# totokunda/apex-studio

Measured on AMD Instinct MI355X. Metric: denoise_steps_per_sec, higher is better.
Workload: dtype bf16; 1 GPU; flux-dev-1024x1024 denoise step (19 double + 38 single MM-DiT blocks, S_img 4096 + S_txt 512, B=1, no CFG) + FlowMatch-Euler step; clips_in_flight=1, parallelism=clip-per-gpu x1

## Files before the change

### apex-studio_amd/build.py

```python
from __future__ import annotations

import hashlib
import os
import shutil
import subprocess
import sys

PKG_DIR = os.path.dirname(os.path.abspath(__file__))
CSRC = os.path.join(PKG_DIR, "csrc")
LIB_NAME = "libapex_mi355.so"
LIB_PATH = os.path.join(PKG_DIR, LIB_NAME)
SOURCES = ["runtime.hip", "gemm.hip", "attention.hip", "attention_masked.hip", "elementwise.hip", "conv.hip"]
ARCH = "gfx950"


def _hipcc() -> str:
    for cand in (os.environ.get("HIPCC"), shutil.which("hipcc"), "/opt/rocm/bin/hipcc"):
        if cand and os.path.exists(cand):
            return cand
    raise RuntimeError("hipcc not found (set HIPCC or install ROCm)")


FLAGS = ["-O3", "-std=c++17", "-fPIC", "-Wno-unused-result"]
if os.environ.get("APEXMI_GEMM_STREAMK", "0") not in ("", "0"):
    FLAGS.append("-DAPEXMI_GEMM_STREAMK=1")
if os.environ.get("APEXMI_DEBUG", "0") not in ("", "0"):
    FLAGS.append("-DAPEXMI_DEBUG")


NO_SPILL = {"attention.hip": ["attn_fwd_d128_w64_kernel", "attn_fwd_d128_w64r_kernel"],
            "attention_masked.hip": ["attn_masked_kernel"]}
REMARKS = "-Rpass-analysis=kernel-resource-usage"


def parse_resource_remarks(text: str) -> dict:
    import re
    out, cur = {}, None
    for line in text.splitlines():
        m = re.search(r"remark:\s+Function Name: (\S+)", line)
        if m:
            cur = out.setdefault(m.group(1), {})
            continue
        m = re.search(r"remark:\s+([A-Za-z ]+?)(?: \[[^\]]*\])?: (\d+)", line)
        if m and cur is not None:
            cur[m.group(1).strip()] = int(m.group(2))
    return out


def check_no_spill(src: str, remarks: str) -> None:
    res = parse_resource_remarks(remarks)
    for want in NO_SPILL.get(src, []):
        hits = {k: v for k, v in res.items() if want in k}
        if not hits:
            raise RuntimeError(f"build: no resource remark for kernel '{want}' of {src} — the spill check cannot run")
        for k, v in hits.items():
            bad = {f: v.get(f, -1) for f in ("ScratchSize", "SGPRs Spill", "VGPRs Spill") if v.get(f, -1) != 0}
            if bad:
                raise RuntimeError(f"build: {k} ({src}) has a hand-fixed register map and must not spill, but the compiler "
                                   f"reports {bad} (VGPRs {v.get('VGPRs')}, AGPRs {v.get('AGPRs')}, SGPRs {v.get('TotalSGPRs')}): "
                                   f"this hipcc allocates differently from the one the map was written against")


def _digest(paths: list[str], extra: str = "") -> str:
    h = hashlib.sha256(extra.encode())
    for p in paths:
        with open(p, "rb") as f:
            h.update(hashlib.sha256(f.read()).digest())
    return h.hexdigest()


def _stale(target: str, digest: str) -> bool:
    stamp = target + ".sha256"
    if not (os.path.exists(target) and os.path.exists(stamp)):
        return True
    with open(stamp) as f:
        return f.read().strip() != digest


def _stamp(target: str, digest: str) -> None:
    with open(target + ".sha256", "w") as f:
        f.write(digest + "\n")


def build(force: bool = False, verbose: bool = True) -> str:
    hipcc = _hipcc()
    headers = [os.path.join(CSRC, "common.h"),
               os.path.join(PKG_DIR, "..", "include", "apexmi.h")]
    headers += sorted(os.path.join(CSRC, f) for f in os.listdir(CSRC) if f.endswith((".inc", ".h")) and f != "common.h")
    objs = []
    jobs = []
    for src in SOURCES:
        sp = os.path.join(CSRC, src)
        op = os.path.join(CSRC, src.replace(".hip", ".o"))
        objs.append(op)
        dg = _digest([sp] + headers, " ".join(FLAGS + ([REMARKS + ":checked"] if src in NO_SPILL else []) + [ARCH]))
        if force or _stale(op, dg):
            cmd = [hipcc, f"--offload-arch={ARCH}", *FLAGS, *([REMARKS] if src in NO_SPILL else []), "-c", sp, "-o", op]
            if verbose:
                print("[build]", " ".join(cmd), flush=True)
            jobs.append((subprocess.Popen(cmd, stderr=subprocess.PIPE if src in NO_SPILL else None, text=True), cmd, op, dg, src))
    for proc, cmd, op, dg, src in jobs:
        err = proc.communicate()[1]
        if err:
            rest = [l for l in err.splitlines() if "kernel-resource-usage" not in l and not l.lstrip().startswith(("|", "^"))
                    and not l.strip()[:1].isdigit() and not l.startswith("In file included from")]
            if rest and verbose:
                print("\n".join(rest), file=sys.stderr, flush=True)
        if proc.returncode != 0:
            if err:
                print(err[-4000:], file=sys.stderr)
            raise subprocess.CalledProcessError(proc.returncode, cmd)
        if src in NO_SPILL:
            check_no_spill(src, err or "")
        _stamp(op, dg)
    dg = _digest(objs, ARCH)
    if force or _stale(LIB_PATH, dg):
        cmd = [hipcc, f"--offload-arch={ARCH}", "-shared", "-fPIC", "-o", LIB_PATH] + objs
        if verbose:
            print("[build]", " ".join(cmd), flush=True)
        subprocess.check_call(cmd)
        _stamp(LIB_PATH, dg)
    return LIB_PATH


if __name__ == "__main__":
    build(force="--force" in sys.argv)
    print(LIB_PATH)
```

### apex-studio_amd/csrc/gemm.hip

```cpp
#include "common.h"

#include <cstring>
#include <mutex>
#include <tuple>
#include <type_traits>
#include <vector>

namespace {

#ifndef APEXMI_GEMM_ABLATE
#define APEXMI_GEMM_ABLATE 0
#endif
#ifndef APEXMI_GEMM_PEEL
#define APEXMI_GEMM_PEEL 2
#endif
#ifndef APEXMI_GEMM_STREAMK
#define APEXMI_GEMM_STREAMK 0
#endif
#ifndef APEXMI_GEMM_TRACE
#define APEXMI_GEMM_TRACE 0
#endif
constexpr int BK = 64;
constexpr int GROUP_M = 6;
constexpr int EPI_GATE_RES_F32 = 7;
constexpr int MAX_GROUPS = 4;

struct GemmProblem {
    const bf16_t* A;
    const bf16_t* W;
    const bf16_t* bias;
    bf16_t* C;
    const float* gate;
    const bf16_t* R;
    int64_t lda, ldw, ldc, ldr;
    int M, N, nm, nn, tile0, gelu;
    int qkv, row0;
    const bf16_t* nq;
    const bf16_t* nk;
};
struct QkvShared {
    bf16_t* qo;
    bf16_t* ko;
    bf16_t* vt;
    const float* rope;
    int S_out, Skp, inner;
    float eps;
    const float* rope_pairs;
};
struct GemmGroup {
    GemmProblem p[MAX_GROUPS];
    int count, K, total, group_m;
    int batch;
    int64_t bsA, bsW, bsC_bytes;
    QkvShared qs;
    unsigned long long* clk;
#if APEXMI_GEMM_TRACE
    unsigned long long* trace;
#endif
    int wpacked;
    int sk_r, sk_tfull;
    float* sk_slab;
    unsigned* sk_flag;
};
enum { TILE_FULL = 0, TILE_WRITER = 1, TILE_OWNER = 2 };
struct SkCtx {
    int mode, kt0, kt1;
    int cu;
    int nparts;
};

template <int BM_, int BN_, int WM_, int WN_, int SCHED_>
struct Cfg {
    static constexpr int BM = BM_, BN = BN_, WM = WM_, WN = WN_;
    static constexpr int SCHED = SCHED_;
    static constexpr bool PP = SCHED_ == 1;
    static constexpr int NW = WM * WN, NT = NW * 64;
    static constexpr int TM = BM / WM / 32, TN = BN / WN / 32;
    static constexpr int A_BYTES = BM * BK * 2, W_BYTES = BN * BK * 2;
    static constexpr int STAGE = A_BYTES + W_BYTES;
    static constexpr int LDS = SCHED_ == 8 ? 5 * 32768 : 2 * STAGE;
    static constexpr int A_LD = BM * 8 / NT, W_LD = BN * 8 / NT;
    static constexpr int OCC = (LDS <= 80 * 1024 && NT == 256) ? 2 : (NT == 512 ? 2 : 1);
};
using CFG_128 = Cfg<128, 128, 2, 2, 0>;
using CFG_256 = Cfg<256, 256, 2, 4, 0>;
using CFG_128E = Cfg<128, 128, 2, 4, 0>;
using CFG_256P = Cfg<256, 256, 2, 4, 1>;
using CFG_256W = Cfg<256, 256, 2, 2, 4>;
using CFG_256P16 = Cfg<256, 256, 2, 4, 5>;
using CFG_256R = Cfg<256, 256, 2, 4, 7>;
using CFG_256R5 = Cfg<256, 256, 2, 4, 8>;

APEXMI_DEVICE float act_f(float x, int mode) {
    if (mode == 1) return gelu_tanh_f(x);
    if (mode == 2) return 0.5f * x * (1.0f + erff(x * 0.70710678118654752f));
    if (mode == 4) return x_sigmoid_log2(x, (1.702f * 1.4426950408889634f) * x);
    return silu_f(x);
}
template <int ACT>
APEXMI_DEVICE float act_c(float x) {
    if constexpr (ACT == 0) return x;
    else return act_f(x, ACT);
}
#define APEXMI_ACT_DISPATCH(mode, ...)                                    \
    switch (mode) {                                                       \
        case 1: { constexpr int ACT = 1; __VA_ARGS__; } break;            \
        case 2: { constexpr int ACT = 2; __VA_ARGS__; } break;            \
        case 3: { constexpr int ACT = 3; __VA_ARGS__; } break;            \
        case 4: { constexpr int ACT = 4; __VA_ARGS__; } break;            \
        default: { constexpr int ACT = 0; __VA_ARGS__; } break;           \
    }
inline int act_mode(int epilogue) {
    return epilogue == APEXMI_EPI_BIAS_GELU ? 1 : epilogue == APEXMI_EPI_BIAS_GELU_ERF ? 2 : epilogue == APEXMI_EPI_BIAS_SILU ? 3 : epilogue == APEXMI_EPI_BIAS_QUICK_GELU ? 4 : 0;
}

APEXMI_DEVICE void swap_pair(u32x2& a, u32x2& b) {
#pragma unroll
    for (int i = 0; i < 2; ++i) {
        auto r = __builtin_amdgcn_permlane32_swap(a[i], b[i], false, false);
        a[i] = r[0];
        b[i] = r[1];
    }
}

template <int EPI, int TM, int ACT = 0>
APEXMI_DEVICE void store_ntile(const f32x16 (&acc)[TM], const GemmProblem& P, int N, const int (&m)[TM],
                               int nbase, int hi) {
    float bs[4][4];
    f32x4 gt[4];
#pragma unroll
    for (int g = 0; g < 4; ++g) {
        const int n = min(nbase + 8 * g + 4 * hi, N - 4);
        u32x2 b = {0u, 0u};
        if (P.bias != nullptr) b = *(const u32x2*)(P.bias + n);
        bs[g][0] = bf16_lo(b[0]);
        bs[g][1] = bf16_hi(b[0]);
        bs[g][2] = bf16_lo(b[1]);
        bs[g][3] = bf16_hi(b[1]);
        if (EPI == APEXMI_EPI_BIAS_GATE_RES || EPI == EPI_GATE_RES_F32) gt[g] = *(const f32x4*)(P.gate + n);
    }
    if (EPI == APEXMI_EPI_BIAS_F32 || EPI == EPI_GATE_RES_F32) {
        float* Cf = (float*)P.C;
        const float* Rf = (const float*)P.R;
#pragma unroll
        for (int mt = 0; mt < TM; ++mt)
#pragma unroll
            for (int g = 0; g < 4; ++g) {
                const int n = nbase + 8 * g + 4 * hi;
                if (m[mt] >= 0 && n < N) {
                    float o[4];
#pragma unroll
                    for (int j = 0; j < 4; ++j) {
                        o[j] = acc[mt][4 * g + j] + bs[g][j];
                        o[j] = act_c<ACT>(o[j]);
                    }
                    if (EPI == EPI_GATE_RES_F32) {
                        const f32x4 r = *(const f32x4*)(Rf + (int64_t)m[mt] * P.ldr + n);
#pragma unroll
                        for (int j = 0; j < 4; ++j) o[j] = r[j] + gt[g][j] * o[j];
                    }
                    *(f32x4*)(Cf + (int64_t)m[mt] * P.ldc + n) = f32x4{o[0], o[1], o[2], o[3]};
                }
            }
        return;
    }
    u32x4 rr[TM][2];
    if (EPI == APEXMI_EPI_BIAS_GATE_RES) {
#pragma unroll
        for (int mt = 0; mt < TM; ++mt)
#pragma unroll
            for (int pr = 0; pr < 2; ++pr) {
                const int nst = min(nbase + 8 * (2 * pr + hi), N - 8);
                rr[mt][pr] = *(const u32x4*)(P.R + (int64_t)max(m[mt], 0) * P.ldr + nst);
            }
    }
#pragma unroll
    for (int mt = 0; mt < TM; ++mt)
#pragma unroll
        for (int pr = 0; pr < 2; ++pr) {
            const int g0 = 2 * pr;
            const int nst = nbase + 8 * (g0 + hi);
            float v[2][4];
#pragma unroll
            for (int q = 0; q < 2; ++q)
#pragma unroll
                for (int j = 0; j < 4; ++j) {
                    v[q][j] = acc[mt][4 * (g0 + q) + j] + bs[g0 + q][j];
                    v[q][j] = act_c<ACT>(v[q][j]);
                }
            if (EPI == APEXMI_EPI_BIAS_GATE_RES) {
                u32x2 ra = {rr[mt][pr][0], rr[mt][pr][1]}, rb = {rr[mt][pr][2], rr[mt][pr][3]};
                swap_pair(ra, rb);
#pragma unroll
                for (int q = 0; q < 2; ++q) {
                    const u32x2 r2 = q ? rb : ra;
                    v[q][0] = bf16_lo(r2[0]) + gt[g0 + q][0] * v[q][0];
                    v[q][1] = bf16_hi(r2[0]) + gt[g0 + q][1] * v[q][1];
                    v[q][2] = bf16_lo(r2[1]) + gt[g0 + q][2] * v[q][2];
                    v[q][3] = bf16_hi(r2[1]) + gt[g0 + q][3] * v[q][3];
                }
            }
            u32x2 oa = {pack_bf16(v[0][0], v[0][1]), pack_bf16(v[0][2], v[0][3])};
            u32x2 ob = {pack_bf16(v[1][0], v[1][1]), pack_bf16(v[1][2], v[1][3])};
            swap_pair(oa, ob);
            if (m[mt] >= 0 && nst < N) {
                const u32x4 o = {oa[0], oa[1], ob[0], ob[1]};
                *(u32x4*)(P.C + (int64_t)m[mt] * P.ldc + nst) = o;
            }
        }
}


typedef __attribute__((ext_vector_type(4))) float f32x4_t;

APEXMI_DEVICE float sum_xor16(float x) {
    auto r = __builtin_amdgcn_permlane16_swap(__float_as_uint(x), __float_as_uint(x), false, false);
    return __uint_as_float(r[0]) + __uint_as_float(r[1]);
}
APEXMI_DEVICE void swap16(uint32_t& a, uint32_t& b) {
    auto r = __builtin_amdgcn_permlane16_swap(a, b, false, false);
    a = r[0];
    b = r[1];
}

template <int EPI, int MT, int ACT = 0>
APEXMI_DEVICE void store_slab16(const f32x4_t (&x)[MT], const f32x4_t (&y)[MT], const GemmProblem& P, int N,
                                const int (&m)[MT], int nbase, int g, const u32x4* rr_pre = nullptr) {
    float bs[2][4];
    f32x4 gt[2];
#pragma unroll
    for (int t = 0; t < 2; ++t) {
        const int n = min(nbase + 16 * t + 4 * g, N - 4);
        u32x2 b = {0u, 0u};
        if (P.bias != nullptr) b = *(const u32x2*)(P.bias + n);
        bs[t][0] = bf16_lo(b[0]);
        bs[t][1] = bf16_hi(b[0]);
        bs[t][2] = bf16_lo(b[1]);
        bs[t][3] = bf16_hi(b[1]);
        if (EPI == APEXMI_EPI_BIAS_GATE_RES || EPI == EPI_GATE_RES_F32) gt[t] = *(const f32x4*)(P.gate + n);
    }
    if (EPI == APEXMI_EPI_BIAS_F32 || EPI == EPI_GATE_RES_F32) {
        float* Cf = (float*)P.C;
        const float* Rf = (const float*)P.R;
#pragma unroll
        for (int mt = 0; mt < MT; ++mt)
#pragma unroll
            for (int t = 0; t < 2; ++t) {
                const int n = nbase + 16 * t + 4 * g;
                const f32x4_t& a = t ? y[mt] : x[mt];
                if (m[mt] >= 0 && n < N) {
                    float o[4];
#pragma unroll
                    for (int j = 0; j < 4; ++j) {
                        o[j] = a[j] + bs[t][j];
                        o[j] = act_c<ACT>(o[j]);
                    }
                    if (EPI == EPI_GATE_RES_F32) {
                        const f32x4 r = *(const f32x4*)(Rf + (int64_t)m[mt] * P.ldr + n);
#pragma unroll
                        for (int j = 0; j < 4; ++j) o[j] = r[j] + gt[t][j] * o[j];
                    }
                    *(f32x4*)(Cf + (int64_t)m[mt] * P.ldc + n) = f32x4{o[0], o[1], o[2], o[3]};
                }
            }
        return;
    }
    const int nst = nbase + 16 * (g & 1) + 8 * (g >> 1);
    u32x4 rr[MT];
    if (EPI == APEXMI_EPI_BIAS_GATE_RES) {
#pragma unroll
        for (int mt = 0; mt < MT; ++mt)
            rr[mt] = rr_pre ? rr_pre[mt] : *(const u32x4*)(P.R + (int64_t)max(m[mt], 0) * P.ldr + min(nst, N - 8));
    }
#pragma unroll
    for (int mt = 0; mt < MT; ++mt) {
        float v[2][4];
#pragma unroll
        for (int j = 0; j < 4; ++j) {
            v[0][j] = x[mt][j] + bs[0][j];
            v[1][j] = y[mt][j] + bs[1][j];
            v[0][j] = act_c<ACT>(v[0][j]);
            v[1][j] = act_c<ACT>(v[1][j]);
        }
        if (EPI == APEXMI_EPI_BIAS_GATE_RES) {
            uint32_t r0 = rr[mt][0], r1 = rr[mt][1], r2 = rr[mt][2], r3 = rr[mt][3];
            swap16(r0, r2);
            swap16(r1, r3);
            const uint32_t ra[2][2] = {{r0, r1}, {r2, r3}};
#pragma unroll
            for (int t = 0; t < 2; ++t) {
                v[t][0] = bf16_lo(ra[t][0]) + gt[t][0] * v[t][0];
                v[t][1] = bf16_hi(ra[t][0]) + gt[t][1] * v[t][1];
                v[t][2] = bf16_lo(ra[t][1]) + gt[t][2] * v[t][2];
                v[t][3] = bf16_hi(ra[t][1]) + gt[t][3] * v[t][3];
            }
        }
        uint32_t x0 = pack_bf16(v[0][0], v[0][1]), x1 = pack_bf16(v[0][2], v[0][3]);
        uint32_t y0 = pack_bf16(v[1][0], v[1][1]), y1 = pack_bf16(v[1][2], v[1][3]);
        swap16(x0, y0);
        swap16(x1, y1);
        if (m[mt] >= 0 && nst < N) {
            const u32x4 o = {x0, x1, y0, y1};
            *(u32x4*)(P.C + (int64_t)m[mt] * P.ldc + nst) = o;
        }
    }
}

#ifndef APEXMI_QK_ABL
#define APEXMI_QK_ABL 0
#endif
template <int MT = 8, int WROWS = 128>
APEXMI_DEVICE void qkv_epilogue16(f32x4_t (&acc16)[4][MT], const GemmProblem& P, const QkvShared& Q, int M, int m0, int n0,
                                  int wave, int wm, int wn, int lane, char* smem) {
    const int g = lane >> 4, c = lane & 15;
    const int which = n0 / Q.inner;
    const int ncol0 = n0 - which * Q.inner;
    float bs[2][4];
    auto load_bias = [&](int p) {
#pragma unroll
        for (int t = 0; t < 2; ++t) {
            u32x2 b = {0u, 0u};
            if (P.bias != nullptr) b = *(const u32x2*)(P.bias + n0 + wn * 64 + p * 32 + 16 * t + 4 * g);
            bs[t][0] = bf16_lo(b[0]);
            bs[t][1] = bf16_hi(b[0]);
            bs[t][2] = bf16_lo(b[1]);
            bs[t][3] = bf16_hi(b[1]);
        }
    };
    auto rounded = [&](int p, int mt) -> u32x4 {
        const f32x4_t& x = acc16[2 * p][mt];
        const f32x4_t& y = acc16[2 * p + 1][mt];
        uint32_t x0 = pack_bf16(x[0] + bs[0][0], x[1] + bs[0][1]), x1 = pack_bf16(x[2] + bs[0][2], x[3] + bs[0][3]);
        uint32_t y0 = pack_bf16(y[0] + bs[1][0], y[1] + bs[1][1]), y1 = pack_bf16(y[2] + bs[1][2], y[3] + bs[1][3]);
        swap16(x0, y0);
        swap16(x1, y1);
        return u32x4{x0, x1, y0, y1};
    };
    const int cw = 16 * (g & 1) + 8 * (g >> 1);
    __syncthreads();
    if (which == 2) {
        constexpr int NPASS = (2 * WROWS * 512 > 160 * 1024) ? 2 : 1;
        constexpr int ROWS = NPASS == 1 ? 2 * WROWS : WROWS;
        bf16_t* tile = (bf16_t*)smem;
        const int tid = wave * 64 + lane;
#pragma unroll
        for (int pass = 0; pass < NPASS; ++pass) {
            if (NPASS == 2 && pass == 1) __syncthreads();
            if (NPASS == 1 || wm == pass) {
#pragma unroll
                for (int p = 0; p < 2; ++p) {
                    load_bias(p);
#pragma unroll
                    for (int mt = 0; mt < MT; ++mt) {
                        const int r = (NPASS == 1 ? wm * WROWS : 0) + mt * 16 + c;
                        const int dch = (wn * 64 + p * 32 + cw) >> 3;
                        *(u32x4*)(tile + r * 256 + (((dch + (r >> 3) + 4 * (r & 7)) & 31) << 3)) = rounded(p, mt);
                    }
                }
            }
            __syncthreads();
            const int mp = m0 + (NPASS == 1 ? 0 : pass * WROWS);
            if (((P.row0 | M) & 7) != 0) {
                for (int i = 0; i < ROWS / 2; ++i) {
                    const int idx = i * 512 + tid;
                    const int r = idx % ROWS, d = idx / ROWS;
                    const bf16_t e = tile[r * 256 + ((((d >> 3) + (r >> 3) + 4 * (r & 7)) & 31) << 3) + (d & 7)];
                    const int h = (ncol0 + d) >> 7, dd = (ncol0 + d) & 127;
                    if (mp + r < M) Q.vt[((int64_t)h * 128 + dd) * Q.Skp + P.row0 + mp + r] = e;
                }
                continue;
            }
#pragma unroll 4
            for (int i = 0; i < ROWS / 16; ++i) {
                const int idx = i * 512 + tid;
                const int sc = idx & 7, d = (idx >> 3) & 255, sc_hi = idx >> 11;
                const int s8 = (sc_hi * 8 + sc) * 8;
                uint32_t w[4];
#pragma unroll
                for (int j = 0; j < 8; ++j) {
                    const int r = s8 + j;
                    const uint32_t e = tile[r * 256 + ((((d >> 3) + (r >> 3) + 4 * (r & 7)) & 31) << 3) + (d & 7)];
                    if (j & 1) w[j >> 1] |= e << 16;
                    else w[j >> 1] = e;
                }
                const int h = (ncol0 + d) >> 7, dd = (ncol0 + d) & 127;
                if (mp + s8 < M)
                    *(u32x4*)(Q.vt + ((int64_t)h * 128 + dd) * Q.Skp + P.row0 + mp + s8) = u32x4{w[0], w[1], w[2], w[3]};
            }
        }
        return;
    }
    float* red = (float*)smem;
#pragma unroll
    for (int p = 0; p < ((APEXMI_QK_ABL & 4) ? 0 : 2); ++p) {
        load_bias(p);
#pragma unroll
        for (int mt = 0; mt < MT; ++mt) {
            float x[8];
            unpack8(rounded(p, mt), x);
            float sq = 0.0f;
#pragma unroll
            for (int j = 0; j < 8; ++j) sq += x[j] * x[j];
            red[(wave * 2 * MT + p * MT + mt) * 64 + lane] = sq;
        }
    }
    __syncthreads();
    const bf16_t* nw = which ? P.nk : P.nq;
    const int h = (ncol0 >> 7) + (wn >> 1);
    bf16_t* dst_base = (which ? Q.ko : Q.qo) + (int64_t)h * Q.S_out * 128;
    auto rinv_of = [&](int mt) -> float {
        const float a0 = red[(wave * 2 * MT + mt) * 64 + lane] + red[((wave ^ 1) * 2 * MT + mt) * 64 + lane];
        const float a1 = red[(wave * 2 * MT + MT + mt) * 64 + lane] + red[((wave ^ 1) * 2 * MT + MT + mt) * 64 + lane];
        float sq = a0 + a1;
        sq = sum_xor16(sq);
        sq = sum_xor32(sq);
        return rsqrtf(sq * (1.0f / 128) + Q.eps);
    };
    float rinv[MT > 8 ? 1 : MT];
    if constexpr (MT <= 8) {
#pragma unroll
        for (int mt = 0; mt < MT; ++mt) rinv[mt] = rinv_of(mt);
    }
    if constexpr (!(APEXMI_QK_ABL & 64)) {
        if (Q.rope_pairs != nullptr) {
            constexpr int NIT = 2 * MT, NS = 5;
            constexpr int RED_BYTES = 8 * 2 * MT * 64 * 4;
            char* ring = smem + RED_BYTES + wave * (NS * 2048);
            const unsigned ring_lane = (unsigned)(uintptr_t)(__attribute__((address_space(3))) char*)ring + (unsigned)lane * 16u;
            auto issue = [&](int it) {
                const int p = it / MT, mt = it % MT;
                const int d = (wn & 1) * 64 + p * 32 + cw;
                int m = m0 + wm * WROWS + mt * 16 + c;
                asm volatile("" : "+v"(m));
                const int srow = P.row0 + min(m, M - 1);
                const float* cp = Q.rope_pairs + (int64_t)srow * 64 + (d >> 1);
                char* dst = ring + (it % NS) * 2048;
                glds16(cp, dst);
                glds16(cp + (int64_t)Q.S_out * 64, dst + 1024);
            };
#pragma unroll
            for (int it = 0; it < NS - 1; ++it) issue(it);
            float* wtab = (float*)(smem + RED_BYTES + 8 * NS * 2048) + wave * 1024 + lane * 8;
            float wv[MT > 8 ? 1 : 8];
            if constexpr (MT > 8) {
                if (nw != nullptr) {
#pragma unroll
                    for (int p = 0; p < 2; ++p) {
                        float w8[8];
                        unpack8(*(const u32x4*)(nw + (wn & 1) * 64 + p * 32 + cw), w8);
                        *(f32x4*)(wtab + p * 512) = f32x4{w8[0], w8[1], w8[2], w8[3]};
                        *(f32x4*)(wtab + p * 512 + 4) = f32x4{w8[4], w8[5], w8[6], w8[7]};
                    }
                }
            }
            auto body = [&](auto IT) {
                constexpr int it = decltype(IT)::value;
                if constexpr (it < NIT) {
                    constexpr int p = it / MT, mt = it % MT;
                    constexpr int later = (NIT - 1 - it) < (NS - 1) ? (NIT - 1 - it) : (NS - 1);
                    if constexpr (it + NS - 1 < NIT) issue(it + NS - 1);
                    const int d = (wn & 1) * 64 + p * 32 + cw;
                    if constexpr (mt == 0) {
                        load_bias(p);
                        if constexpr (MT <= 8) {
                            if (nw != nullptr) unpack8(*(const u32x4*)(nw + d), wv);
                        }
                    }
                    float x[8], y[8];
                    unpack8(rounded(p, mt), x);
                    if (nw != nullptr) {
                        if constexpr (MT > 8) {
                            const float ri = rinv_of(mt);
                            const f32x4 w0 = *(const f32x4*)(wtab + p * 512), w1 = *(const f32x4*)(wtab + p * 512 + 4);
#pragma unroll
                            for (int j = 0; j < 4; ++j) {
                                x[j] = x[j] * ri * w0[j];
                                x[j + 4] = x[j + 4] * ri * w1[j];
                            }
                        } else {
                            const float ri = rinv[MT > 8 ? 0 : mt];
#pragma unroll
                            for (int j = 0; j < 8; ++j) x[j] = x[j] * ri * wv[MT > 8 ? 0 : j];
                        }
                    }
                    f32x4 cq, sq4;
                    asm volatile("s_waitcnt vmcnt(%3)\n\t"
                                 "ds_read_b128 %0, %2 offset:%4\n\t"
                                 "ds_read_b128 %1, %2 offset:%5\n\t"
                                 "s_waitcnt lgkmcnt(0)"
                                 : "=&v"(cq), "=&v"(sq4)
                                 : "v"(ring_lane), "n"(2 * later), "n"((it % NS) * 2048), "n"((it % NS) * 2048 + 1024)
                                 : "memory");
#pragma unroll
                    for (int q = 0; q < 4; ++q) {
                        y[2 * q] = fmaf(x[2 * q], cq[q], -(x[2 * q + 1] * sq4[q]));
                        y[2 * q + 1] = fmaf(x[2 * q + 1], cq[q], x[2 * q] * sq4[q]);
                    }
                    int m = m0 + wm * WROWS + mt * 16 + c;
                    asm volatile("" : "+v"(m));
                    const int srow = P.row0 + min(m, M - 1);
                    if (m < M)
                        *(u32x4*)(dst_base + (int64_t)srow * 128 + d) =
                            u32x4{pack_bf16(y[0], y[1]), pack_bf16(y[2], y[3]), pack_bf16(y[4], y[5]), pack_bf16(y[6], y[7])};
                    __builtin_amdgcn_sched_barrier(0);
                }
            };
#define APEXMI_QK_IT(i) body(std::integral_constant<int, (i)>{});
            APEXMI_QK_IT(0) APEXMI_QK_IT(1) APEXMI_QK_IT(2) APEXMI_QK_IT(3) APEXMI_QK_IT(4) APEXMI_QK_IT(5)
            APEXMI_QK_IT(6) APEXMI_QK_IT(7) APEXMI_QK_IT(8) APEXMI_QK_IT(9) APEXMI_QK_IT(10) APEXMI_QK_IT(11)
            APEXMI_QK_IT(12) APEXMI_QK_IT(13) APEXMI_QK_IT(14) APEXMI_QK_IT(15) APEXMI_QK_IT(16) APEXMI_QK_IT(17)
            APEXMI_QK_IT(18) APEXMI_QK_IT(19) APEXMI_QK_IT(20) APEXMI_QK_IT(21) APEXMI_QK_IT(22) APEXMI_QK_IT(23)
#undef APEXMI_QK_IT
            static_assert(NIT <= 24, "the unrolled call list above covers 24 iterations");
            static_assert(MT > 8 ? RED_BYTES + 8 * NS * 2048 + 8 * 4096 <= 160 * 1024 : RED_BYTES + 8 * NS * 2048 <= 128 * 1024,
                          "sums + ring (+ weights) must fit the tile's LDS");
            return;
        }
    }
#pragma unroll
    for (int p = 0; p < ((APEXMI_QK_ABL & 32) ? 0 : 2); ++p) {
        const int d = (wn & 1) * 64 + p * 32 + cw;
        load_bias(p);
        float wv[8];
        if (nw != nullptr) unpack8(*(const u32x4*)(nw + d), wv);
#pragma unroll
        for (int mt = 0; mt < MT; ++mt) {
            const int m = m0 + wm * WROWS + mt * 16 + c;
            const int srow = P.row0 + min(m, M - 1);
            float x[8], y[8];
            unpack8(rounded(p, mt), x);
            if (nw != nullptr) {
                const float ri = (APEXMI_QK_ABL & 8) ? 1.0f : MT > 8 ? rinv_of(mt) : rinv[MT > 8 ? 0 : mt];
#pragma unroll
                for (int j = 0; j < 8; ++j) x[j] = x[j] * ri * wv[j];
            }
            const float* cp = Q.rope + (int64_t)srow * 128 + d;
            const float* sp = Q.rope + (int64_t)Q.S_out * 128 + (int64_t)srow * 128 + d;
            float cs[8], sn[8];
            if constexpr (APEXMI_QK_ABL & 1) {
#pragma unroll
                for (int j = 0; j < 8; ++j) cs[j] = 1.f, sn[j] = 0.5f;
            } else {
                const f32x4 c0 = *(const f32x4*)cp, c1 = *(const f32x4*)(cp + 4);
                const f32x4 s0 = *(const f32x4*)sp, s1 = *(const f32x4*)(sp + 4);
#pragma unroll
                for (int j = 0; j < 4; ++j) {
                    cs[j] = c0[j];
                    cs[j + 4] = c1[j];
                    sn[j] = s0[j];
                    sn[j + 4] = s1[j];
                }
            }
#pragma unroll
            for (int q = 0; q < 4; ++q) {
                y[2 * q] = fmaf(x[2 * q], cs[2 * q], -(x[2 * q + 1] * sn[2 * q]));
                y[2 * q + 1] = fmaf(x[2 * q + 1], cs[2 * q + 1], x[2 * q] * sn[2 * q + 1]);
            }
            if ((APEXMI_QK_ABL & 2) ? (y[0] + y[3] + y[5] == 12345.678f) : (m < M))
                *(u32x4*)(dst_base + (int64_t)srow * 128 + d) =
                    u32x4{pack_bf16(y[0], y[1]), pack_bf16(y[2], y[3]), pack_bf16(y[4], y[5]), pack_bf16(y[6], y[7])};
            if (!(APEXMI_QK_ABL & 16) && (MT > 8 || (mt & 1))) __builtin_amdgcn_sched_barrier(0);
        }
    }
}

#if APEXMI_GEMM_TRACE
#define APEXMI_TRACE_END()                                                                                   \
    do {                                                                                                     \
        if (G.trace != nullptr) {                                                                            \
            __builtin_amdgcn_sched_barrier(0);                                                               \
            const unsigned long long t_st = __builtin_amdgcn_s_memrealtime();                                \
            asm volatile("s_waitcnt vmcnt(0)" ::: "memory");                                                 \
            const unsigned long long t_ack = __builtin_amdgcn_s_memrealtime();                               \
            if (tid == 0) {                                                                                  \
                unsigned long long* o = G.trace + (size_t)blockIdx.x * 8;                                    \
                o[0] = __builtin_amdgcn_s_getreg((31 << 11) | (0 << 6) | 4);               \
                o[1] = __builtin_amdgcn_s_getreg((31 << 11) | (0 << 6) | 20);             \
                o[2] = tr_in;                                                                                \
                o[3] = tr_l0;                                                                                \
                o[4] = tr_l1;                                                                                \
                o[5] = t_st;                                                                                 \
                o[6] = t_ack;                                                                                \
                o[7] = (unsigned long long)s;                                                                \
            }                                                                                                \
        }                                                                                                    \
    } while (0)
#else
#define APEXMI_TRACE_END() do { } while (0)
#endif

template <typename CFG, int EPI>
__device__ __forceinline__ void gemm_tile(const GemmGroup& G, char* smem, int s, const SkCtx& sk) {
    constexpr int BM = CFG::BM, BN = CFG::BN, TM = CFG::TM, TN = CFG::TN;

#if APEXMI_GEMM_TRACE
    unsigned long long tr_in = 0, tr_l0 = 0, tr_l1 = 0;
    if (G.trace != nullptr) tr_in = __builtin_amdgcn_s_memrealtime();
#endif
    int tid_ = threadIdx.x;
    asm volatile("" : "+v"(tid_));
    const int tid = tid_;
    const int lane = tid & 63;
    const int wave = __builtin_amdgcn_readfirstlane(tid >> 6);
    const int wm = wave / CFG::WN, wn = wave % CFG::WN;
    const int l31 = lane & 31, hi = lane >> 5;

    int gi = 0;
#pragma unroll
    for (int i = 1; i < MAX_GROUPS; ++i)
        if (i < G.count && s >= G.p[i].tile0) gi = i;
    GemmProblem P = G.p[gi];
    if (G.batch > 1) {
        const int64_t z = blockIdx.y;
        P.A += z * G.bsA;
        P.W += z * G.bsW;
        P.C = (bf16_t*)((char*)P.C + z * G.bsC_bytes);
    }
    s -= P.tile0;
    const int nn = P.nn, N = P.N, M = P.M;
    const int GM = G.group_m;
    const int width = GM * nn;
    const int first_m = (s / width) * GM;
    const int gsz = min(P.nm - first_m, GM);
    const int pm = first_m + (s % width) % gsz;
    const int pn = (s % width) / gsz;
    const int m0 = pm * BM, n0 = pn * BN;

    const char* a_src[CFG::A_LD];
    const char* w_src[CFG::W_LD];
#pragma unroll
    for (int i = 0; i < CFG::A_LD; ++i) {
        const int p = (i * CFG::NW + wave) * 64 + lane;
        const int row = p >> 3, c = (p & 7) ^ ((row >> 1) & 7);
        a_src[i] = (const char*)(P.A + (int64_t)min(m0 + row, M - 1) * P.lda + c * 8);
    }
#pragma unroll
    for (int i = 0; i < CFG::W_LD; ++i) {
        const int p = (i * CFG::NW + wave) * 64 + lane;
        const int row = p >> 3, c = (p & 7) ^ ((row >> 1) & 7);
        w_src[i] = (const char*)(P.W + (int64_t)min(n0 + row, N - 1) * P.ldw + c * 8);
    }

    f32x16 acc[TN][TM];
#pragma unroll
    for (int i = 0; i < TN; ++i)
#pragma unroll
        for (int j = 0; j < TM; ++j)
#pragma unroll
            for (int r = 0; r < 16; ++r) acc[i][j][r] = 0.0f;

    f32x4_t acc16[4][8];
    if constexpr (CFG::SCHED == 5 || CFG::SCHED >= 7) {
#pragma unroll
        for (int i = 0; i < 4; ++i)
#pragma unroll
            for (int j = 0; j < 8; ++j) {
                acc16[i][j] = f32x4_t{0.f, 0.f, 0.f, 0.f};
                asm volatile("" : "+v"(acc16[i][j]));
            }
    }
    const int nkt_all = G.K / BK;
    const int nkt = (CFG::SCHED == 5) ? sk.kt1 - sk.kt0 : nkt_all;
    unsigned long long clk_c0 = 0, clk_r0 = 0;
    if (G.clk != nullptr) {
        clk_c0 = __builtin_readcyclecounter();
        clk_r0 = __builtin_amdgcn_s_memrealtime();
    }
#if APEXMI_GEMM_TRACE
    if (G.trace != nullptr) tr_l0 = __builtin_amdgcn_s_memrealtime();
#endif

    auto stage = [&](int buf, int kt) {
        char* base = smem + buf * CFG::STAGE + wave * 1024;
        const int64_t koff = (int64_t)kt * (BK * 2);
#pragma unroll
        for (int i = 0; i < CFG::A_LD; ++i) glds16(a_src[i] + koff, base + i * (CFG::NW * 1024));
#pragma unroll
        for (int i = 0; i < CFG::W_LD; ++i)
            glds16(w_src[i] + koff, base + CFG::A_BYTES + i * (CFG::NW * 1024));
    };

    int a_off[TM], a_sw[TM], w_off[TN], w_sw[TN];
#pragma unroll
    for (int t = 0; t < TM; ++t) {
        const int r = wm * (BM / CFG::WM) + t * 32 + l31;
        a_off[t] = r * 128;
        a_sw[t] = (r >> 1) & 7;
    }
#pragma unroll
    for (int t = 0; t < TN; ++t) {
        const int r = wn * (BN / CFG::WN) + t * 32 + l31;
        w_off[t] = r * 128;
        w_sw[t] = (r >> 1) & 7;
    }

    if constexpr (CFG::SCHED == 0) {
#if APEXMI_GEMM_PEEL >= 2 && !defined(APEXMI_GEMM_SMALL_VECTOR)
        const uint64_t a_u64 = (uint64_t)(P.A + (int64_t)min(m0, M - 1) * P.lda), w_u64 = (uint64_t)(P.W + (int64_t)min(n0, N - 1) * P.ldw);
        const char* const a_u = (const char*)(((uint64_t)(uint32_t)__builtin_amdgcn_readfirstlane((uint32_t)(a_u64 >> 32)) << 32) |
                                              (uint32_t)__builtin_amdgcn_readfirstlane((uint32_t)a_u64));
        const char* const w_u = (const char*)(((uint64_t)(uint32_t)__builtin_amdgcn_readfirstlane((uint32_t)(w_u64 >> 32)) << 32) |
                                              (uint32_t)__builtin_amdgcn_readfirstlane((uint32_t)w_u64));
        uint32_t a_o[CFG::A_LD], w_o[CFG::W_LD];
#pragma unroll
        for (int i = 0; i < CFG::A_LD; ++i) a_o[i] = (uint32_t)(a_src[i] - a_u);
#pragma unroll
        for (int i = 0; i < CFG::W_LD; ++i) w_o[i] = (uint32_t)(w_src[i] - w_u);
        const uint32_t smem_lds0 = __builtin_amdgcn_readfirstlane((uint32_t)(uintptr_t)(__attribute__((address_space(3))) void*)smem);
#pragma clang diagnostic push
#pragma clang diagnostic ignored "-Winline-asm"
        auto piece = [&](const char* sbase, uint32_t voff, uint32_t la) {
            asm volatile("s_mov_b32 m0, %2\n\ts_nop 0\n\tglobal_load_lds_dwordx4 %0, %1"
                         :: "v"(voff), "s"(sbase), "s"(la) : "memory", "m0");
        };
#pragma clang diagnostic pop
        auto stage = [&](int buf, int kt) {
            const uint32_t base = smem_lds0 + buf * CFG::STAGE + wave * 1024;
            const char* ga = a_u + (int64_t)kt * (BK * 2);
            const char* gw = w_u + (int64_t)kt * (BK * 2);
#pragma unroll
            for (int i = 0; i < CFG::A_LD; ++i) piece(ga, a_o[i], base + i * (CFG::NW * 1024));
#pragma unroll
            for (int i = 0; i < CFG::W_LD; ++i) piece(gw, w_o[i], base + CFG::A_BYTES + i * (CFG::NW * 1024));
        };
#endif
        stage(0, 0);
        for (int kt = 0; kt < nkt; ++kt) {
            asm volatile("s_waitcnt vmcnt(0)" ::: "memory");
            __syncthreads();
            if (kt + 1 < nkt) stage((kt + 1) & 1, kt + 1);
            const char* As = smem + (kt & 1) * CFG::STAGE;
            const char* Ws = As + CFG::A_BYTES;
#pragma unroll
            for (int ks = 0; ks < 4; ++ks) {
                const int c = ks * 2 + hi;
                bf16x8 af[TM], wf[TN];
#pragma unroll
                for (int t = 0; t < TM; ++t) af[t] = *(const bf16x8*)(As + a_off[t] + ((c ^ a_sw[t]) << 4));
#pragma unroll
                for (int t = 0; t < TN; ++t) wf[t] = *(const bf16x8*)(Ws + w_off[t] + ((c ^ w_sw[t]) << 4));
#pragma unroll
                for (int nt = 0; nt < TN; ++nt)
#pragma unroll
                    for (int mt = 0; mt < TM; ++mt)
                        acc[nt][mt] = __builtin_amdgcn_mfma_f32_32x32x16_bf16(wf[nt], af[mt], acc[nt][mt], 0, 0, 0);
            }
        }
    } else if constexpr (CFG::SCHED == 4) {
        static_assert(CFG::SCHED != 4 || (TM == 4 && TN == 4 && CFG::NW == 4), "SCHED 4 is written for 2x2 waves of 128x128");
        bf16x8 fa[2][4], fw[2][4];
        const int rows_a = min(M - m0, BM), rows_w = min(N - n0, BN);
        auto rsrc_a = __builtin_amdgcn_make_buffer_rsrc((void*)(P.A + (int64_t)m0 * P.lda), 0,
                                                        (int)(((int64_t)(rows_a - 1) * P.lda + G.K) * 2), 0x00020000);
        auto rsrc_w = __builtin_amdgcn_make_buffer_rsrc((void*)(P.W + (int64_t)n0 * P.ldw), 0,
                                                        (int)(((int64_t)(rows_w - 1) * P.ldw + G.K) * 2), 0x00020000);
        const int sw_src = ((lane & 7) ^ (4 * (wave & 1) + (lane >> 4))) * 16;
        const int voff_a = (lane >> 3) * (int)P.lda * 2 + sw_src;
        const int voff_w = (lane >> 3) * (int)P.ldw * 2 + sw_src;
        const int sa = (int)P.lda * 2 * 8, sw = (int)P.ldw * 2 * 8;
        const int krot = (G.K * 2) % 8192 == 0 ? (int)(blockIdx.x & 7) * (nkt >> 3) : 0;
        auto dma1 = [&](int slot, int kt_, int i) {
            int kt = kt_ + krot;
            kt = kt >= nkt ? kt - nkt : kt;
            char* base = smem + slot * CFG::STAGE + wave * 1024;
            if (i < 8)
                __builtin_amdgcn_raw_ptr_buffer_load_lds(rsrc_a, (__attribute__((address_space(3))) void*)(base + i * 4096), 16, voff_a,
                                                         (i * 4 + wave) * sa + kt * (BK * 2), 0, 0);
            else
                __builtin_amdgcn_raw_ptr_buffer_load_lds(rsrc_w, (__attribute__((address_space(3))) void*)(base + CFG::A_BYTES + (i - 8) * 4096), 16,
                                                         voff_w, ((i - 8) * 4 + wave) * sw + kt * (BK * 2), 0, 0);
        };
        auto rd1 = [&](int slot, int ks, int b, int j) {
            const char* As = smem + slot * CFG::STAGE;
            const char* Ws = As + CFG::A_BYTES;
            const int c = ks * 2 + hi;
            if (j == 0) fw[b][0] = *(const bf16x8*)(Ws + w_off[0] + ((c ^ w_sw[0]) << 4));
            else if (j <= 4) fa[b][j - 1] = *(const bf16x8*)(As + a_off[j - 1] + ((c ^ a_sw[j - 1]) << 4));
            else fw[b][j - 4] = *(const bf16x8*)(Ws + w_off[j - 4] + ((c ^ w_sw[j - 4]) << 4));
        };
        auto mma1 = [&](int b, int i) {
            acc[i >> 2][i & 3] =
                __builtin_amdgcn_mfma_f32_32x32x16_bf16(fw[b][i >> 2], fa[b][i & 3], acc[i >> 2][i & 3], 0, 0, 0);
        };
#define W4_FENCE() __builtin_amdgcn_sched_barrier(0)
        constexpr int ROT = 0;
        constexpr int STEP = 2;
        auto period = [&](int kt, auto has_dma, auto has_next) {
            constexpr bool DMA = decltype(has_dma)::value, NEXT = decltype(has_next)::value;
            const int cur = kt & 1, nxt = cur ^ 1;
            asm volatile("s_waitcnt vmcnt(0) lgkmcnt(0)" ::: "memory");
            W4_FENCE();
            __builtin_amdgcn_s_barrier();
            W4_FENCE();
#pragma unroll
            for (int s = 0; s < (NEXT ? 64 : 16); ++s) {
                const int q = s >> 4, i = s & 15;
                mma1((q + 1) & 1, i);
                if (NEXT && i < 8) rd1(nxt, q, q & 1, i);
                if (DMA && s >= ROT && (s - ROT) % STEP == 0 && (s - ROT) / STEP < 16) dma1(cur, kt + 2, (s - ROT) / STEP);
                W4_FENCE();
            }
        };
#pragma unroll
        for (int i = 0; i < 16; ++i) dma1(0, 0, i);
        if (nkt > 1) {
#pragma unroll
            for (int i = 0; i < 16; ++i) dma1(1, 1, i);
            asm volatile("s_waitcnt vmcnt(16)" ::: "memory");
        } else {
            asm volatile("s_waitcnt vmcnt(0)" ::: "memory");
        }
        W4_FENCE();
        __builtin_amdgcn_s_barrier();
        W4_FENCE();
#pragma unroll
        for (int j = 0; j < 8; ++j) rd1(0, 0, 0, j);
        W4_FENCE();
#pragma unroll
        for (int s = 0; s < 48; ++s) {
            const int q = s >> 4, i = s & 15;
            mma1(q & 1, i);
            if (i < 8) rd1(0, q + 1, (q + 1) & 1, i);
            W4_FENCE();
        }
        int kt = 0;
        for (; kt + 2 < nkt; ++kt) period(kt, std::true_type{}, std::true_type{});
        if (kt + 1 < nkt) {
            period(kt, std::false_type{}, std::true_type{});
            ++kt;
        }
        period(kt, std::false_type{}, std::false_type{});
#undef W4_FENCE
    } else if constexpr (CFG::SCHED >= 7) {
        const int l15 = lane & 15, g4 = lane >> 4;
        const int swz = (g4 ^ (l15 >> 2)) << 4;
        const int rd_a = (wm * 128 + l15) * 64 + swz;
        const int rd_w = 16384 + (wn * 64 + l15) * 64 + swz;
        const char* base_a = (const char*)(P.A + (int64_t)m0 * P.lda);
        const char* base_w = (const char*)(P.W + (int64_t)n0 * P.ldw);
        unsigned off[4];
        int dst[4];
#pragma unroll
        for (int j = 0; j < 2; ++j) {
            const int pc = wave + 8 * j;
            const int row = pc * 16 + (lane >> 2);
            const int c = (lane & 3) ^ ((row >> 2) & 3);
            off[j] = (unsigned)((min(m0 + row, M - 1) - m0) * (int)P.lda * 2 + c * 16);
            off[2 + j] = (unsigned)((min(n0 + row, N - 1) - n0) * (int)P.ldw * 2 + c * 16);
            dst[j] = pc * 1024;
            dst[2 + j] = 16384 + pc * 1024;
        }
        constexpr int RD_ = CFG::SCHED == 8 ? 4 : 3;
        constexpr int NSLOT = RD_ + 1;
        auto dma = [&](int st, int slot) {
            char* base = smem + slot * 32768;
            const char* ka = base_a + (int64_t)st * 64;
            const char* kw = base_w + (int64_t)st * 64;
#pragma unroll
            for (int j = 0; j < 2; ++j) glds16(ka + off[j], base + dst[j]);
#pragma unroll
            for (int j = 2; j < 4; ++j) glds16(kw + off[j], base + dst[j]);
        };
        bf16x8 fa[2][8], fw[2][4];
#define RING_DSR(dstreg, addr, offs) asm volatile("ds_read_b128 %0, %1 offset:%2" : "=v"(dstreg) : "v"(addr), "i"(offs) : "memory")
#define RING_RD(slotidx, set)                              \
    do {                                                   \
        const int slot_ = (slotidx) * 32768;               \
        const int aw_ = slot_ + rd_w, aa_ = slot_ + rd_a;  \
        RING_DSR(fw[set][0], aw_, 0);                      \
        RING_DSR(fw[set][1], aw_, 1024);                   \
        RING_DSR(fw[set][2], aw_, 2048);                   \
        RING_DSR(fw[set][3], aw_, 3072);                   \
        RING_DSR(fa[set][0], aa_, 0);                      \
        RING_DSR(fa[set][1], aa_, 1024);                   \
        RING_DSR(fa[set][2], aa_, 2048);                   \
        RING_DSR(fa[set][3], aa_, 3072);                   \
        RING_DSR(fa[set][4], aa_, 4096);                   \
        RING_DSR(fa[set][5], aa_, 5120);                   \
        RING_DSR(fa[set][6], aa_, 6144);                   \
        RING_DSR(fa[set][7], aa_, 7168);                   \
    } while (0)
#define RING_WAIT(n, set)                                                                                                    \
    asm volatile("s_waitcnt lgkmcnt(" #n ")"                                                                                 \
                 : "+v"(fw[set][0]), "+v"(fw[set][1]), "+v"(fw[set][2]), "+v"(fw[set][3]), "+v"(fa[set][0]), "+v"(fa[set][1]), \
                   "+v"(fa[set][2]), "+v"(fa[set][3]), "+v"(fa[set][4]), "+v"(fa[set][5]), "+v"(fa[set][6]), "+v"(fa[set][7]) \
                 :                                                                                                           \
                 : "memory")
#define RING_MMA(set)                                                                                                      \
    do {                                                                                                                   \
        __builtin_amdgcn_s_setprio(1);                                                                                     \
        _Pragma("unroll") for (int u = 0; u < 4; ++u) _Pragma("unroll") for (int t = 0; t < 8; ++t) acc16[u][t] =          \
            __builtin_amdgcn_mfma_f32_16x16x32_bf16(fw[set][u], fa[set][t], acc16[u][t], 0, 0, 0);                         \
        __builtin_amdgcn_s_setprio(0);                                                                                     \
    } while (0)
#define RING_FENCE() __builtin_amdgcn_sched_barrier(0)
#define RING_VM(n)                                                                       \
    do {                                                                                 \
        if (!(APEXMI_GEMM_ABLATE & 2)) asm volatile("s_waitcnt vmcnt(" #n ")" ::: "memory"); \
    } while (0)
#define RING_BAR()                                                      \
    do {                                                                \
        if (!(APEXMI_GEMM_ABLATE & 1)) __builtin_amdgcn_s_barrier();    \
    } while (0)
#define RING_STEP(st_, set, RD, DMA)                                        \
    do {                                                                    \
        RING_FENCE();                                                       \
        if (RD && !(APEXMI_GEMM_ABLATE & 8)) RING_RD(s_rd, (set) ^ 1);      \
        RING_FENCE();                                                       \
        if (DMA && !(APEXMI_GEMM_ABLATE & 4)) dma((st_) + RD_, s_dma);      \
        RING_FENCE();                                                       \
        if (DMA) {                                                          \
            if (RD_ == 3) RING_VM(4);                                       \
            else RING_VM(8);                                                \
        } else {                                                            \
            RING_VM(0);                                                     \
        }                                                                   \
        RING_FENCE();                                                       \
        RING_BAR();                                                         \
        RING_FENCE();                                                       \
        RING_MMA(set);                                                      \
        if (RD) RING_WAIT(0, (set) ^ 1);                                    \
        RING_FENCE();                                                       \
        RING_BAR();                                                         \
        RING_FENCE();                                                       \
        s_rd = s_rd + 1 == NSLOT ? 0 : s_rd + 1;                            \
        s_dma = s_dma + 1 == NSLOT ? 0 : s_dma + 1;                         \
    } while (0)
        const int ns = nkt * 2;
#pragma unroll
        for (int i = 0; i < RD_; ++i)
            if (i < ns) dma(i, i);
        if (ns >= 4 && RD_ == 4) RING_VM(8);
        else if (ns >= 3) RING_VM(4);
        else RING_VM(0);
        RING_FENCE();
        __builtin_amdgcn_s_barrier();
        RING_FENCE();
        RING_RD(0, 0);
        RING_WAIT(0, 0);
        RING_FENCE();
        if (wm == 1) RING_BAR();
        RING_FENCE();
        int s_rd = 1, s_dma = RD_ % NSLOT;
        int st = 0;
        for (; st + 1 + RD_ < ns; st += 2) {
            RING_STEP(st, 0, true, true);
            RING_STEP(st + 1, 1, true, true);
        }
        if (st + 4 <= ns) {
            if constexpr (RD_ == 3) RING_STEP(st, 0, true, true);
            else RING_STEP(st, 0, true, false);
            RING_STEP(st + 1, 1, true, false);
            st += 2;
        }
        RING_STEP(st, 0, true, false);
        RING_STEP(st + 1, 1, false, false);
        RING_FENCE();
        if (wm == 0) RING_BAR();
        RING_FENCE();
#undef RING_VM
#undef RING_BAR
#undef RING_STEP
#undef RING_MMA
#undef RING_RD
#undef RING_FENCE
#undef RING_DSR
#undef RING_WAIT
    } else if constexpr (CFG::SCHED == 5) {
        const int l15 = lane & 15, g4 = lane >> 4;
        const int sw16 = (l15 >> 1) & 7;
        int a16[8], w16[4];
#pragma unroll
        for (int t = 0; t < 8; ++t) a16[t] = (wm * 128 + t * 16 + l15) * 128;
#pragma unroll
        for (int t = 0; t < 4; ++t) w16[t] = (wn * 64 + t * 16 + l15) * 128;
        const int ch16[2] = {((0 + g4) ^ sw16) << 4, ((4 + g4) ^ sw16) << 4};
        bf16x8 af[4][2], wf[2][2][2];
        auto rd_a = [&](const char* As, int half) {
#pragma unroll
            for (int t = 0; t < 4; ++t)
#pragma unroll
                for (int ks = 0; ks < 2; ++ks) af[t][ks] = *(const bf16x8*)(As + a16[half * 4 + t] + ch16[ks]);
        };
        auto rd_w = [&](const char* Ws, int nt) {
#pragma unroll
            for (int u = 0; u < 2; ++u)
#pragma unroll
                for (int ks = 0; ks < 2; ++ks) wf[nt][u][ks] = *(const bf16x8*)(Ws + w16[nt * 2 + u] + ch16[ks]);
        };
        auto mma = [&](int half, int nt) {
            __builtin_amdgcn_s_setprio(1);
#pragma unroll
            for (int ks = 0; ks < 2; ++ks)
#pragma unroll
                for (int u = 0; u < 2; ++u)
#pragma unroll
                    for (int t = 0; t < 4; ++t)
                        acc16[nt * 2 + u][half * 4 + t] = __builtin_amdgcn_mfma_f32_16x16x32_bf16(
                            wf[nt][u][ks], af[t][ks], acc16[nt * 2 + u][half * 4 + t], 0, 0, 0);
            __builtin_amdgcn_s_setprio(0);
        };
#define PP_SYNC()                                                                   \
    do {                                                                            \
        asm volatile("s_waitcnt lgkmcnt(0)" ::: "memory");                          \
        __builtin_amdgcn_sched_barrier(0);                                          \
        __builtin_amdgcn_s_barrier();                                               \
        __builtin_amdgcn_sched_barrier(0);                                          \
    } while (0)
#define PP_BAR()                               \
    do {                                       \
        __builtin_amdgcn_sched_barrier(0);     \
        __builtin_amdgcn_s_barrier();          \
        __builtin_amdgcn_sched_barrier(0);     \
    } while (0)
        const char* ra_src[2][2];
        const char* rw_src[2][2];
        int ra_row[2][2], rw_row[2][2];
#pragma unroll
        for (int reg = 0; reg < 2; ++reg)
#pragma unroll
            for (int j = 0; j < 2; ++j) {
                const int q = j * 8 + wave;
                const int ra0 = (q < 8 ? q * 8 : 128 + (q - 8) * 8) + reg * 64;
                const int rw0 = (q >> 2) * 64 + reg * 32 + (q & 3) * 8;
                const int ra = ra0 + (lane >> 3), rw = rw0 + (lane >> 3);
                ra_src[reg][j] = (G.wpacked & 2)
                    ? (const char*)(P.A + ((int64_t)pm * nkt_all * 256 + ra) * 64 + (((lane & 7) ^ ((ra >> 1) & 7)) * 8))
                    : (const char*)(P.A + (int64_t)min(m0 + ra, M - 1) * P.lda + (((lane & 7) ^ ((ra >> 1) & 7)) * 8));
                rw_src[reg][j] = (G.wpacked & 1)
                    ? (const char*)(P.W + ((int64_t)pn * nkt_all * 256 + rw) * 64 + (((lane & 7) ^ ((rw >> 1) & 7)) * 8))
                    : (const char*)(P.W + (int64_t)min(n0 + rw, N - 1) * P.ldw + (((lane & 7) ^ ((rw >> 1) & 7)) * 8));
                ra_row[reg][j] = ra0;
                rw_row[reg][j] = rw0;
            }
        const int64_t w_kstep = (G.wpacked & 1) ? 256 * 128 : BK * 2;
        const int64_t a_kstep = (G.wpacked & 2) ? 256 * 128 : BK * 2;
        if (sk.kt0) {
#pragma unroll
            for (int reg = 0; reg < 2; ++reg)
#pragma unroll
                for (int j = 0; j < 2; ++j) {
                    ra_src[reg][j] += (int64_t)sk.kt0 * a_kstep;
                    rw_src[reg][j] += (int64_t)sk.kt0 * w_kstep;
                }
        }
#if APEXMI_GEMM_PEEL >= 2
        auto uniform_ptr = [](const char* p) {
            const uint64_t u = (uint64_t)p;
            const uint32_t lo = __builtin_amdgcn_readfirstlane((uint32_t)u), hi = __builtin_amdgcn_readfirstlane((uint32_t)(u >> 32));
            return (const char*)(((uint64_t)hi << 32) | lo);
        };
        const char* const a_base_u = uniform_ptr((G.wpacked & 2) ? (const char*)(P.A + (int64_t)pm * nkt_all * 256 * 64)
                                                                 : (const char*)(P.A + (int64_t)min(m0, M - 1) * P.lda));
        const char* const w_base_u = uniform_ptr((G.wpacked & 1) ? (const char*)(P.W + (int64_t)pn * nkt_all * 256 * 64)
                                                                 : (const char*)(P.W + (int64_t)min(n0, N - 1) * P.ldw));
        uint32_t ra_off[2][2], rw_off[2][2];
#pragma unroll
        for (int reg = 0; reg < 2; ++reg)
#pragma unroll
            for (int j = 0; j < 2; ++j) {
                ra_off[reg][j] = (uint32_t)(ra_src[reg][j] - a_base_u);
                rw_off[reg][j] = (uint32_t)(rw_src[reg][j] - w_base_u);
            }
        const uint32_t smem_lds = __builtin_amdgcn_readfirstlane((uint32_t)(uintptr_t)(__attribute__((address_space(3))) void*)smem);
#pragma clang diagnostic push
#pragma clang diagnostic ignored "-Winline-asm"
        auto glds16_s = [&](const char* sbase, uint32_t voff, uint32_t la) {
            asm volatile("s_mov_b32 m0, %2\n\ts_nop 0\n\tglobal_load_lds_dwordx4 %0, %1"
                         :: "v"(voff), "s"(sbase), "s"(la) : "memory", "m0");
        };
#pragma clang diagnostic pop
        auto stage_a = [&](int buf, int kt, int reg) {
            const uint32_t base = smem_lds + buf * CFG::STAGE;
            const char* gb = a_base_u + (int64_t)kt * a_kstep;
#pragma unroll
            for (int j = 0; j < 2; ++j) glds16_s(gb, ra_off[reg][j], base + ra_row[reg][j] * 128);
        };
        auto stage_w = [&](int buf, int kt, int reg) {
            const uint32_t base = smem_lds + buf * CFG::STAGE + CFG::A_BYTES;
            const char* gb = w_base_u + (int64_t)kt * w_kstep;
#pragma unroll
            for (int j = 0; j < 2; ++j) glds16_s(gb, rw_off[reg][j], base + rw_row[reg][j] * 128);
        };
#else
        auto stage_a = [&](int buf, int kt, int reg) {
            char* base = smem + buf * CFG::STAGE;
#pragma unroll
            for (int j = 0; j < 2; ++j) {
                glds16(ra_src[reg][j] + (int64_t)kt * a_kstep, base + ra_row[reg][j] * 128);
            }
        };
        auto stage_w = [&](int buf, int kt, int reg) {
            char* base = smem + buf * CFG::STAGE + CFG::A_BYTES;
#pragma unroll
            for (int j = 0; j < 2; ++j) {
                glds16(rw_src[reg][j] + (int64_t)kt * w_kstep, base + rw_row[reg][j] * 128);
            }
        };
#endif
#define VMCNT(n) asm volatile("s_waitcnt vmcnt(" #n ")" ::: "memory")
        stage_a(0, 0, 0);
        stage_w(0, 0, 0);
        stage_w(0, 0, 1);
        stage_a(0, 0, 1);
        VMCNT(0);
        PP_BAR();
        if (wm == 1) PP_BAR();
        auto ktile = [&](int kt, auto more_c) {
            constexpr bool more = decltype(more_c)::value;
            const char* As = smem + (kt & 1) * CFG::STAGE;
            const char* Ws = As + CFG::A_BYTES;
            const int nb = (kt + 1) & 1;
            rd_a(As, 0);
            rd_w(Ws, 0);
            if constexpr (more) { stage_a(nb, kt + 1, 0); VMCNT(4); } else { VMCNT(2); }
            PP_SYNC();
            mma(0, 0);
            PP_BAR();
            rd_w(Ws, 1);
            if constexpr (more) { stage_w(nb, kt + 1, 0); VMCNT(4); } else { VMCNT(0); }
            PP_SYNC();
            mma(0, 1);
            PP_BAR();
            rd_a(As, 1);
            if constexpr (more) { stage_w(nb, kt + 1, 1); VMCNT(4); }
            PP_SYNC();
            mma(1, 1);
            PP_BAR();
            if constexpr (more) { stage_a(nb, kt + 1, 1); VMCNT(4); }
            PP_SYNC();
            mma(1, 0);
            PP_BAR();
        };
        for (int kt = 0; kt + 1 < nkt; ++kt) ktile(kt, std::true_type{});
        if (nkt > 0) ktile(nkt - 1, std::false_type{});
        if (wm == 0) PP_BAR();
#undef VMCNT
#undef PP_SYNC
#undef PP_BAR
    } else {
        static_assert(!CFG::PP || (TM == 4 && TN == 2), "ping-pong schedule is written for 128x64 wave tiles");
        bf16x8 af[2][4], wf[4];
        auto rd_a = [&](const char* As, int half) {
#pragma unroll
            for (int t = 0; t < 2; ++t)
#pragma unroll
                for (int ks = 0; ks < 4; ++ks)
                    af[t][ks] = *(const bf16x8*)(As + a_off[half * 2 + t] + (((ks * 2 + hi) ^ a_sw[half * 2 + t]) << 4));
        };
        auto rd_w = [&](const char* Ws, int nt) {
#pragma unroll
            for (int ks = 0; ks < 4; ++ks)
                wf[ks] = *(const bf16x8*)(Ws + w_off[nt] + (((ks * 2 + hi) ^ w_sw[nt]) << 4));
        };
        auto mma = [&](int half, int nt) {
            __builtin_amdgcn_s_setprio(1);
#pragma unroll
            for (int ks = 0; ks < 4; ++ks)
#pragma unroll
                for (int t = 0; t < 2; ++t)
                    acc[nt][half * 2 + t] =
                        __builtin_amdgcn_mfma_f32_32x32x16_bf16(wf[ks], af[t][ks], acc[nt][half * 2 + t], 0, 0, 0);
            __builtin_amdgcn_s_setprio(0);
        };
#define PP_SYNC()                                                                   \
    do {                                                                            \
        asm volatile("s_waitcnt lgkmcnt(0)" ::: "memory");                          \
        __builtin_amdgcn_sched_barrier(0);                                          \
        __builtin_amdgcn_s_barrier();                                               \
        __builtin_amdgcn_sched_barrier(0);                                          \
    } while (0)
#define PP_BAR()                               \
    do {                                       \
        __builtin_amdgcn_sched_barrier(0);     \
        __builtin_amdgcn_s_barrier();          \
        __builtin_amdgcn_sched_barrier(0);     \
    } while (0)

        const char* ra_src[2][2];
        const char* rw_src[2][2];
        int ra_lds[2][2], rw_lds[2][2];
#pragma unroll
        for (int reg = 0; reg < 2; ++reg)
#pragma unroll
            for (int j = 0; j < 2; ++j) {
                const int q = j * 8 + wave;
                const int ra0 = (q < 8 ? q * 8 : 128 + (q - 8) * 8) + reg * 64;
                const int rw0 = (q >> 2) * 64 + reg * 32 + (q & 3) * 8;
                const int ra = ra0 + (lane >> 3), rw = rw0 + (lane >> 3);
                ra_src[reg][j] = (const char*)(P.A + (int64_t)min(m0 + ra, M - 1) * P.lda + (((lane & 7) ^ ((ra >> 1) & 7)) * 8));
                rw_src[reg][j] = (const char*)(P.W + (int64_t)min(n0 + rw, N - 1) * P.ldw + (((lane & 7) ^ ((rw >> 1) & 7)) * 8));
                ra_lds[reg][j] = ra0 * 128;
                rw_lds[reg][j] = CFG::A_BYTES + rw0 * 128;
            }
        auto stage_a = [&](int buf, int kt, int reg) {
            char* base = smem + buf * CFG::STAGE;
            const int64_t koff = (int64_t)kt * (BK * 2);
#pragma unroll
            for (int j = 0; j < 2; ++j) glds16(ra_src[reg][j] + koff, base + ra_lds[reg][j]);
        };
        auto stage_w = [&](int buf, int kt, int reg) {
            char* base = smem + buf * CFG::STAGE;
            const int64_t koff = (int64_t)kt * (BK * 2);
#pragma unroll
            for (int j = 0; j < 2; ++j) glds16(rw_src[reg][j] + koff, base + rw_lds[reg][j]);
        };
#define VMCNT(n) asm volatile("s_waitcnt vmcnt(" #n ")" ::: "memory")

        stage_a(0, 0, 0);
        stage_w(0, 0, 0);
        stage_w(0, 0, 1);
        stage_a(0, 0, 1);
        VMCNT(0);
        PP_BAR();
        if (wm == 1) PP_BAR();
        for (int kt = 0; kt < nkt; ++kt) {
            const char* As = smem + (kt & 1) * CFG::STAGE;
            const char* Ws = As + CFG::A_BYTES;
            const bool more = kt + 1 < nkt;
            const int nb = (kt + 1) & 1;
            rd_a(As, 0);
            rd_w(Ws, 0);
            if (more) stage_a(nb, kt + 1, 0);
            if (more) { VMCNT(4); } else { VMCNT(2); }
            PP_SYNC();
            mma(0, 0);
            PP_BAR();
            rd_w(Ws, 1);
            if (more) stage_w(nb, kt + 1, 0);
            if (more) { VMCNT(4); } else { VMCNT(0); }
            PP_SYNC();
            mma(0, 1);
            PP_BAR();
            rd_a(As, 1);
            if (more) stage_w(nb, kt + 1, 1);
            if (more) VMCNT(4);
            PP_SYNC();
            mma(1, 1);
            PP_BAR();
            rd_w(Ws, 0);
            if (more) stage_a(nb, kt + 1, 1);
            if (more) VMCNT(4);
            PP_SYNC();
            mma(1, 0);
            PP_BAR();
        }
        if (wm == 0) PP_BAR();
#undef VMCNT
#undef PP_SYNC
#undef PP_BAR
    }

#if APEXMI_GEMM_TRACE
    if (G.trace != nullptr) {
        __builtin_amdgcn_sched_barrier(0);
        tr_l1 = __builtin_amdgcn_s_memrealtime();
        __builtin_amdgcn_sched_barrier(0);
    }
#endif
    if (G.clk != nullptr) {
        const unsigned long long c1 = __builtin_readcyclecounter(), r1 = __builtin_amdgcn_s_memrealtime();
        if (tid == 0) {
            atomicAdd(G.clk, c1 - clk_c0);
            atomicAdd(G.clk + 1, r1 - clk_r0);
        }
    }

    if constexpr (CFG::SCHED == 5 && APEXMI_GEMM_STREAMK) {
        typedef __attribute__((ext_vector_type(4))) unsigned int u32x4_;
        if (sk.mode == TILE_WRITER) {
            auto rs = __builtin_amdgcn_make_buffer_rsrc((void*)(G.sk_slab + (size_t)sk.cu * 65536), 0, 262144, 0x00020000);
#pragma unroll
            for (int i = 0; i < 4; ++i)
#pragma unroll
                for (int j = 0; j < 8; ++j)
                    __builtin_amdgcn_raw_buffer_store_b128(__builtin_bit_cast(u32x4_, acc16[i][j]), rs, tid * 16, (i * 8 + j) * 8192, 16);
            asm volatile("s_waitcnt vmcnt(0)" ::: "memory");
            __syncthreads();
            if (tid == 0) __hip_atomic_store(G.sk_flag + sk.cu, 1u, __ATOMIC_RELAXED, __HIP_MEMORY_SCOPE_AGENT);
            return;
        }
        if (sk.mode == TILE_OWNER) {
            if (tid == 0)
                for (int p = 1; p <= sk.nparts; ++p)
                    while (__hip_atomic_load(G.sk_flag + sk.cu - p, __ATOMIC_RELAXED, __HIP_MEMORY_SCOPE_AGENT) == 0u) __builtin_amdgcn_s_sleep(2);
            __syncthreads();
            for (int p = 1; p <= sk.nparts; ++p) {
                auto rs = __builtin_amdgcn_make_buffer_rsrc((void*)(G.sk_slab + (size_t)(sk.cu - p) * 65536), 0, 262144, 0x00020000);
#pragma unroll
                for (int i = 0; i < 4; ++i) {
                    u32x4_ v[8];
#pragma unroll
                    for (int j = 0; j < 8; ++j) v[j] = __builtin_amdgcn_raw_buffer_load_b128(rs, tid * 16, (i * 8 + j) * 8192, 16);
#pragma unroll
                    for (int j = 0; j < 8; ++j) acc16[i][j] += __builtin_bit_cast(f32x4_t, v[j]);
                    __builtin_amdgcn_sched_barrier(0);
                }
            }
            __syncthreads();
            if (tid == 0)
                for (int p = 1; p <= sk.nparts; ++p) __hip_atomic_store(G.sk_flag + sk.cu - p, 0u, __ATOMIC_RELAXED, __HIP_MEMORY_SCOPE_AGENT);
        }
    }

    if constexpr (CFG::SCHED == 5 || CFG::SCHED >= 7) {
        if constexpr (EPI == APEXMI_EPI_BIAS) {
            if (P.qkv) {
                qkv_epilogue16(acc16, P, G.qs, M, m0, n0, wave, wm, wn, lane, smem);
                APEXMI_TRACE_END();
                return;
            }
        }
        int mrow16[8];
#pragma unroll
        for (int mt = 0; mt < 8; ++mt) {
            mrow16[mt] = m0 + wm * 128 + mt * 16 + (lane & 15);
            if (mrow16[mt] >= M) mrow16[mt] = -1;
        }
        if constexpr (EPI == APEXMI_EPI_BIAS_GATE_RES) {
            u32x4 rr2[2][8];
            const int g = lane >> 4;
#pragma unroll
            for (int p = 0; p < 2; ++p) {
                const int nst = n0 + wn * 64 + p * 32 + 16 * (g & 1) + 8 * (g >> 1);
#pragma unroll
                for (int mt = 0; mt < 8; ++mt)
                    rr2[p][mt] = *(const u32x4*)(P.R + (int64_t)max(mrow16[mt], 0) * P.ldr + min(nst, N - 8));
            }
#pragma unroll
            for (int p = 0; p < 2; ++p)
                store_slab16<EPI, 8, 0>(acc16[2 * p], acc16[2 * p + 1], P, N, mrow16, n0 + wn * 64 + p * 32, g, rr2[p]);
        } else {
            APEXMI_ACT_DISPATCH((EPI == APEXMI_EPI_BIAS || EPI == APEXMI_EPI_BIAS_F32) ? P.gelu : 0,
                                _Pragma("unroll") for (int p = 0; p < 2; ++p)
                                    store_slab16<EPI, 8, ACT>(acc16[2 * p], acc16[2 * p + 1], P, N, mrow16, n0 + wn * 64 + p * 32, lane >> 4));
        }
        APEXMI_TRACE_END();
        return;
    }
    int mrow[TM];
#pragma unroll
    for (int mt = 0; mt < TM; ++mt) {
        mrow[mt] = m0 + wm * (BM / CFG::WM) + mt * 32 + l31;
        if (mrow[mt] >= M) mrow[mt] = -1;
    }
    APEXMI_ACT_DISPATCH((EPI == APEXMI_EPI_BIAS || EPI == APEXMI_EPI_BIAS_F32) ? P.gelu : 0,
                        _Pragma("unroll") for (int nt = 0; nt < TN; ++nt)
                            store_ntile<EPI, TM, ACT>(acc[nt], P, N, mrow, n0 + wn * (BN / CFG::WN) + nt * 32, hi));
}

template <typename CFG, int EPI>
__global__ __launch_bounds__(CFG::NT, CFG::OCC) void gemm_bf16_kernel(const GemmGroup G) {
    extern __shared__ __attribute__((aligned(16))) char smem[];
    const int nkt = G.K / BK;
    SkCtx sk{TILE_FULL, 0, nkt, 0, 0};
    if constexpr (CFG::SCHED != 5) {
        gemm_tile<CFG, EPI>(G, smem, xcd_remap(blockIdx.x, G.total), sk);
    } else {
        if (!APEXMI_GEMM_STREAMK || (G.sk_r <= 0 && G.sk_tfull <= 0)) {
            gemm_tile<CFG, EPI>(G, smem, xcd_remap(blockIdx.x, G.total), sk);
            return;
        }
        for (int it = 0;; ++it) {
            int bid = blockIdx.x;
            asm volatile("" : "+s"(bid));
            const int x = bid & 7, i = bid >> 3;
            const int rx = G.sk_r / 8 + (x < G.sk_r % 8 ? 1 : 0);
            const int r0 = G.sk_tfull + x * (G.sk_r / 8) + min(x, G.sk_r % 8);
            const int64_t units = (int64_t)rx * nkt;
            auto ustart = [&](int w) { return (int)((units * w) / 32); };
            const int u0 = ustart(i), u1 = ustart(i + 1);
            int j0 = 0, j1 = -1;
            if (u1 > u0) {
                j0 = u0 / nkt;
                j1 = (u1 - 1) / nkt;
            }
            const bool has_head = u1 > u0 && u1 < (j1 + 1) * nkt;
            const bool has_tail = u1 > u0 && u0 > j0 * nkt && !(has_head && j0 == j1);
            const int w_lo = j0 + ((u1 > u0 && u0 > j0 * nkt) ? 1 : 0);
            const int w_hi = j1 - (has_head ? 1 : 0);
            const int n_whole = max(w_hi - w_lo + 1, 0);
            const int per_xcd = G.sk_tfull / 8;
            const int n_full = per_xcd > i ? (per_xcd - i + 31) / 32 : 0;
            const int n_items = (has_head ? 1 : 0) + n_whole + n_full + (has_tail ? 1 : 0);
            if (it >= n_items) break;
            int k = it, tile;
            sk.mode = TILE_FULL;
            sk.kt0 = 0;
            sk.kt1 = nkt;
            sk.nparts = 0;
            sk.cu = x * 32 + i;
            if (has_head && k == 0) {
                sk.mode = TILE_WRITER;
                sk.kt0 = max(u0, j1 * nkt) - j1 * nkt;
                sk.kt1 = u1 - j1 * nkt;
                tile = r0 + j1;
            } else {
                k -= has_head ? 1 : 0;
                if (k < n_whole) {
                    tile = r0 + w_lo + k;
                } else if (k < n_whole + n_full) {
                    tile = x * per_xcd + i + 32 * (k - n_whole);
                } else {
                    sk.mode = TILE_OWNER;
                    sk.kt0 = u0 - j0 * nkt;
                    sk.kt1 = min(u1, (j0 + 1) * nkt) - j0 * nkt;
                    for (int w = i - 1; w >= 0 && sk.nparts < 3; --w) {
                        if (ustart(w + 1) <= j0 * nkt) break;
                        ++sk.nparts;
                    }
                    tile = r0 + j0;
                }
            }
            if (it) __syncthreads();
            gemm_tile<CFG, EPI>(G, smem, tile, sk);
        }
    }
}

__global__ __launch_bounds__(256) void split_bf16x3_kernel(const float* __restrict__ x, int64_t ldx, int64_t M, int K,
                                                            bf16_t* __restrict__ out, int64_t ldo) {
    const int kc = K >> 3;
    const int64_t idx = (int64_t)blockIdx.x * 256 + threadIdx.x;
    if (idx >= M * kc) return;
    const int64_t m = idx / kc;
    const int c = (int)(idx % kc) * 8;
    float v[8], h[8], md[8], lo[8];
    load8<float>(x + m * ldx + c, v);
#pragma unroll
    for (int j = 0; j < 8; ++j) {
        h[j] = bf16_to_f32(f32_to_bf16(v[j]));
        const float r1 = v[j] - h[j];
        md[j] = bf16_to_f32(f32_to_bf16(r1));
        lo[j] = r1 - md[j];
    }
    bf16_t* o = out + m * ldo + c;
    store8<bf16_t>(o, h);
    store8<bf16_t>(o + K, md);
    store8<bf16_t>(o + 2 * (int64_t)K, lo);
}

constexpr int XBM = 288, XBN = 192;
constexpr int X_A_BYTES = XBM * BK * 2, X_W_BYTES = XBN * BK * 2, X_STAGE = X_A_BYTES + X_W_BYTES, X_LDS = 2 * X_STAGE;

template <int EPI, int MT, int ACT = 0>
APEXMI_DEVICE void store_single16(const f32x4_t (&x)[MT], const GemmProblem& P, int N, const int (&m)[MT], int nb, int g,
                                  const u32x2* rr_pre) {
    const int nl = min(nb + 4 * g, N - 4);
    float bs[4] = {0.f, 0.f, 0.f, 0.f};
    if (P.bias != nullptr) {
        const u32x2 b = *(const u32x2*)(P.bias + nl);
        bs[0] = bf16_lo(b[0]);
        bs[1] = bf16_hi(b[0]);
        bs[2] = bf16_lo(b[1]);
        bs[3] = bf16_hi(b[1]);
    }
    f32x4 gt = {0.f, 0.f, 0.f, 0.f};
    if (EPI == APEXMI_EPI_BIAS_GATE_RES) gt = *(const f32x4*)(P.gate + nl);
#pragma unroll
    for (int mt = 0; mt < MT; ++mt) {
        float v[4];
#pragma unroll
        for (int j = 0; j < 4; ++j) v[j] = act_c<ACT>(x[mt][j] + bs[j]);
        if (EPI == APEXMI_EPI_BIAS_GATE_RES) {
            const u32x2 r = rr_pre[mt];
            v[0] = bf16_lo(r[0]) + gt[0] * v[0];
            v[1] = bf16_hi(r[0]) + gt[1] * v[1];
            v[2] = bf16_lo(r[1]) + gt[2] * v[2];
            v[3] = bf16_hi(r[1]) + gt[3] * v[3];
        }
        if (m[mt] >= 0 && nb + 4 * g < N)
            *(u32x2*)(P.C + (int64_t)m[mt] * P.ldc + nb + 4 * g) = u32x2{pack_bf16(v[0], v[1]), pack_bf16(v[2], v[3])};
    }
}

template <int EPI>
__global__ __launch_bounds__(512, 2) void gemm_bf16_x288_kernel(const GemmGroup G) {
    extern __shared__ __attribute__((aligned(16))) char smem[];
    const int tid = threadIdx.x;
    const int lane = tid & 63;
    const int wave = __builtin_amdgcn_readfirstlane(tid >> 6);
    const int wm = wave >> 2, wn = wave & 3;

    int s = xcd_remap(blockIdx.x, G.total);
    int gi = 0;
#pragma unroll
    for (int i = 1; i < MAX_GROUPS; ++i)
        if (i < G.count && s >= G.p[i].tile0) gi = i;
    const GemmProblem P = G.p[gi];
    s -= P.tile0;
    const int nn = P.nn, N = P.N, M = P.M;
    const int GM = G.group_m;
    const int width = GM * nn;
    const int first_m = (s / width) * GM;
    const int gsz = min(P.nm - first_m, GM);
    const int pm = first_m + (s % width) % gsz;
    const int pn = (s % width) / gsz;
    const int m0 = pm * XBM, n0 = pn * XBN;

    const char* src[8];
    int dst[8];
#pragma unroll
    for (int j = 0; j < 8; ++j) {
        int row0;
        bool isw = false;
        if (j < 3) {
            isw = true;
            row0 = (j * 8 + wave) * 8;
        } else if (j < 5) {
            const int q = (j - 3) * 8 + wave;
            row0 = q < 6 ? q * 8 : q < 12 ? 144 + (q - 6) * 8 : (q - 12) * 8;
        } else {
            const int q = (j - 5) * 8 + wave;
            row0 = q < 6 ? 48 + q * 8 : q < 12 ? 192 + (q - 6) * 8 : q < 18 ? 96 + (q - 12) * 8 : 240 + (q - 18) * 8;
        }
        const int row = row0 + (lane >> 3);
        const int c = (lane & 7) ^ ((row >> 1) & 7);
        src[j] = isw ? (const char*)(P.W + (int64_t)min(n0 + row, N - 1) * P.ldw + c * 8)
                     : (const char*)(P.A + (int64_t)min(m0 + row, M - 1) * P.lda + c * 8);
        dst[j] = (isw ? X_A_BYTES : 0) + row0 * 128;
    }
    auto stage = [&](int buf, int kt, int j) { glds16(src[j] + (int64_t)kt * (BK * 2), smem + buf * X_STAGE + dst[j]); };

    f32x4_t acc[3][9];
#pragma unroll
    for (int i = 0; i < 3; ++i)
#pragma unroll
        for (int j = 0; j < 9; ++j) acc[i][j] = f32x4_t{0.f, 0.f, 0.f, 0.f};

    const int nkt = G.K / BK;
    unsigned long long clk_c0 = 0, clk_r0 = 0;
    if (G.clk != nullptr) {
        clk_c0 = __builtin_readcyclecounter();
        clk_r0 = __builtin_amdgcn_s_memrealtime();
    }

    const int l15 = lane & 15, g4 = lane >> 4;
    const int sw16 = (l15 >> 1) & 7;
    const int a_base = (wm * 144 + l15) * 128, w_base = X_A_BYTES + (wn * 48 + l15) * 128;
    const int ch16[2] = {((0 + g4) ^ sw16) << 4, ((4 + g4) ^ sw16) << 4};
    bf16x8 af[3][2], wf[3][2];
    auto rd_a = [&](const char* St, int grp) {
#pragma unroll
        for (int t = 0; t < 3; ++t)
#pragma unroll
            for (int ks = 0; ks < 2; ++ks) af[t][ks] = *(const bf16x8*)(St + a_base + (grp * 3 + t) * 2048 + ch16[ks]);
    };
    auto rd_w = [&](const char* St) {
#pragma unroll
        for (int t = 0; t < 3; ++t)
#pragma unroll
            for (int ks = 0; ks < 2; ++ks) wf[t][ks] = *(const bf16x8*)(St + w_base + t * 2048 + ch16[ks]);
    };
    auto mma = [&](int grp) {
        __builtin_amdgcn_s_setprio(1);
#pragma unroll
        for (int ks = 0; ks < 2; ++ks)
#pragma unroll
            for (int nt = 0; nt < 3; ++nt)
#pragma unroll
                for (int t = 0; t < 3; ++t)
                    acc[nt][grp * 3 + t] =
                        __builtin_amdgcn_mfma_f32_16x16x32_bf16(wf[nt][ks], af[t][ks], acc[nt][grp * 3 + t], 0, 0, 0);
        __builtin_amdgcn_s_setprio(0);
    };
#define X_SYNC()                                                                    \
    do {                                                                            \
        asm volatile("s_waitcnt lgkmcnt(0)" ::: "memory");                          \
        __builtin_amdgcn_sched_barrier(0);                                          \
        __builtin_amdgcn_s_barrier();                                               \
        __builtin_amdgcn_sched_barrier(0);                                          \
    } while (0)
#define X_BAR()                                \
    do {                                       \
        __builtin_amdgcn_sched_barrier(0);     \
        __builtin_amdgcn_s_barrier();          \
        __builtin_amdgcn_sched_barrier(0);     \
    } while (0)
#define X_VMCNT(n) asm volatile("s_waitcnt vmcnt(" #n ")" ::: "memory")
#pragma unroll
    for (int j = 0; j < 8; ++j) stage(0, 0, j);
    X_VMCNT(0);
    X_BAR();
    if (wm == 1) X_BAR();
    for (int kt = 0; kt < nkt; ++kt) {
        const char* St = smem + (kt & 1) * X_STAGE;
        const bool more = kt + 1 < nkt;
        const int nb = (kt + 1) & 1;
        rd_w(St);
        rd_a(St, 0);
        if (more) {
            stage(nb, kt + 1, 0);
            stage(nb, kt + 1, 1);
            stage(nb, kt + 1, 2);
            X_VMCNT(4);
        } else {
            X_VMCNT(1);
        }
        X_SYNC();
        mma(0);
        X_BAR();
        rd_a(St, 1);
        if (more) {
            stage(nb, kt + 1, 3);
            stage(nb, kt + 1, 4);
            stage(nb, kt + 1, 5);
            X_VMCNT(6);
        } else {
            X_VMCNT(0);
        }
        X_SYNC();
        mma(1);
        X_BAR();
        rd_a(St, 2);
        if (more) {
            stage(nb, kt + 1, 6);
            stage(nb, kt + 1, 7);
            X_VMCNT(3);
        }
        X_SYNC();
        mma(2);
        X_BAR();
    }
    if (wm == 0) X_BAR();
#undef X_VMCNT
#undef X_SYNC
#undef X_BAR

    if (G.clk != nullptr) {
        const unsigned long long c1 = __builtin_readcyclecounter(), r1 = __builtin_amdgcn_s_memrealtime();
        if (tid == 0) {
            atomicAdd(G.clk, c1 - clk_c0);
            atomicAdd(G.clk + 1, r1 - clk_r0);
        }
    }

    int mrow[9];
#pragma unroll
    for (int mt = 0; mt < 9; ++mt) {
        mrow[mt] = m0 + wm * 144 + mt * 16 + l15;
        if (mrow[mt] >= M) mrow[mt] = -1;
    }
    const int nbase = n0 + wn * 48;
    if constexpr (EPI == APEXMI_EPI_BIAS_GATE_RES) {
        u32x4 rr[9];
        u32x2 r1[9];
        const int nst = nbase + 16 * (g4 & 1) + 8 * (g4 >> 1);
#pragma unroll
        for (int mt = 0; mt < 9; ++mt) {
            const bf16_t* row = P.R + (int64_t)max(mrow[mt], 0) * P.ldr;
            rr[mt] = *(const u32x4*)(row + min(nst, N - 8));
            r1[mt] = *(const u32x2*)(row + min(nbase + 32 + 4 * g4, N - 4));
        }
        store_slab16<EPI, 9, 0>(acc[0], acc[1], P, N, mrow, nbase, g4, rr);
        store_single16<EPI, 9, 0>(acc[2], P, N, mrow, nbase + 32, g4, r1);
    } else {
        APEXMI_ACT_DISPATCH(P.gelu, store_slab16<EPI, 9, ACT>(acc[0], acc[1], P, N, mrow, nbase, g4);
                            store_single16<EPI, 9, ACT>(acc[2], P, N, mrow, nbase + 32, g4, nullptr));
    }
}

constexpr int YBM = 384, YBN = 256;
constexpr int Y_A_BYTES = YBM * BK * 2, Y_W_BYTES = YBN * BK * 2, Y_STAGE = Y_A_BYTES + Y_W_BYTES, Y_LDS = 2 * Y_STAGE;

template <int EPI, int DIST = 1, int QKV = 0>
__global__ __launch_bounds__(512, 2) void gemm_bf16_x384_kernel(const GemmGroup G) {
    extern __shared__ __attribute__((aligned(16))) char smem[];
    const int tid = threadIdx.x;
    const int lane = tid & 63;
    const int wave = __builtin_amdgcn_readfirstlane(tid >> 6);
    const int wm = wave >> 2, wn = wave & 3;

    int s = xcd_remap(blockIdx.x, G.total);
    int gi = 0;
#pragma unroll
    for (int i = 1; i < MAX_GROUPS; ++i)
        if (i < G.count && s >= G.p[i].tile0) gi = i;
    const GemmProblem P = G.p[gi];
    s -= P.tile0;
    const int nn = P.nn, N = P.N, M = P.M;
    const int GM = G.group_m;
    const int width = GM * nn;
    const int first_m = (s / width) * GM;
    const int gsz = min(P.nm - first_m, GM);
    const int pm = first_m + (s % width) % gsz;
    const int pn = (s % width) / gsz;
    const int m0 = pm * YBM, n0 = pn * YBN;

    const int rows_a = min(M - m0, YBM), rows_w = min(N - n0, YBN);
    auto rsrc_a = __builtin_amdgcn_make_buffer_rsrc((void*)(P.A + (int64_t)m0 * P.lda), 0,
                                                    (int)(((int64_t)(rows_a - 1) * P.lda + G.K) * 2), 0x00020000);
    auto rsrc_w = __builtin_amdgcn_make_buffer_rsrc((void*)(P.W + (int64_t)n0 * P.ldw), 0,
                                                    (int)(((int64_t)(rows_w - 1) * P.ldw + G.K) * 2), 0x00020000);
    const int par = wave & 1, widx = wave >> 1;
    const int sw_src = ((lane & 7) ^ (4 * par + (lane >> 4))) * 16;
    const int voff_a = (lane >> 3) * (int)P.lda * 2 + sw_src;
    const int voff_w = (lane >> 3) * (int)P.ldw * 2 + sw_src;
    const int lda8 = (int)P.lda * 16, ldw8 = (int)P.ldw * 16;
    auto piece_of = [&](int j) -> int {
        if (j < 4) return 2 * (4 * j + widx) + par;
        const int e = 3 * widx + (j < 7 ? j - 4 : j - 7);
        return (e < 6 ? 0 : 24) + (j < 7 ? 0 : 12) + 2 * (e % 6) + par;
    };
    auto stage = [&](int buf, int kt, int j) {
        const int pc = piece_of(j);
        char* dst = smem + buf * Y_STAGE + (j < 4 ? Y_A_BYTES : 0) + pc * 1024;
        if (j < 4)
            __builtin_amdgcn_raw_ptr_buffer_load_lds(rsrc_w, (__attribute__((address_space(3))) void*)dst, 16, voff_w, pc * ldw8 + kt * (BK * 2), 0, 0);
        else
            __builtin_amdgcn_raw_ptr_buffer_load_lds(rsrc_a, (__attribute__((address_space(3))) void*)dst, 16, voff_a, pc * lda8 + kt * (BK * 2), 0, 0);
    };

    f32x4_t acc[4][12];
#pragma unroll
    for (int i = 0; i < 4; ++i)
#pragma unroll
        for (int j = 0; j < 12; ++j) acc[i][j] = f32x4_t{0.f, 0.f, 0.f, 0.f};

    const int nkt = G.K / BK;
    unsigned long long clk_c0 = 0, clk_r0 = 0;
    if (G.clk != nullptr) {
        clk_c0 = __builtin_readcyclecounter();
        clk_r0 = __builtin_amdgcn_s_memrealtime();
    }
#if APEXMI_GEMM_TRACE
    const unsigned long long y_t_in = G.trace != nullptr ? __builtin_amdgcn_s_memrealtime() : 0;
    unsigned long long y_t_loop = 0;
#define Y_TRACE_END(kind)                                                                                   \
    do {                                                                                                    \
        if (G.trace != nullptr) {                                                                           \
            asm volatile("s_waitcnt vmcnt(0)" ::: "memory");                                                \
            __syncthreads();                                                                                \
            if (tid == 0) {                                                                                 \
                unsigned long long* o = G.trace + (size_t)blockIdx.x * 4;                                   \
                o[0] = (unsigned long long)(kind);                                                          \
                o[1] = y_t_in;                                                                              \
                o[2] = y_t_loop;                                                                            \
                o[3] = __builtin_amdgcn_s_memrealtime();                                                    \
            }                                                                                               \
        }                                                                                                   \
    } while (0)
#else
#define Y_TRACE_END(kind) do { } while (0)
#endif

    const int l15 = lane & 15, g4 = lane >> 4;
    const int sw16 = (l15 >> 1) & 7;
    const int a_base = (wm * 192 + l15) * 128, w_base = Y_A_BYTES + (wn * 64 + l15) * 128;
    const int ch16[2] = {((0 + g4) ^ sw16) << 4, ((4 + g4) ^ sw16) << 4};
    bf16x8 af[6], wf[4];
    auto rd_a = [&](const char* St, int h, int ks) {
#pragma unroll
        for (int t = 0; t < 6; ++t) af[t] = *(const bf16x8*)(St + a_base + (h * 6 + t) * 2048 + ch16[ks]);
    };
    auto rd_w = [&](const char* St, int ks) {
#pragma unroll
        for (int t = 0; t < 4; ++t) wf[t] = *(const bf16x8*)(St + w_base + t * 2048 + ch16[ks]);
    };
    auto mma = [&](int h) {
        __builtin_amdgcn_s_setprio(1);
#pragma unroll
        for (int nt = 0; nt < 4; ++nt)
#pragma unroll
            for (int t = 0; t < 6; ++t)
                acc[nt][h * 6 + t] = __builtin_amdgcn_mfma_f32_16x16x32_bf16(wf[nt], af[t], acc[nt][h * 6 + t], 0, 0, 0);
        __builtin_amdgcn_s_setprio(0);
    };
#define Y_SYNC()                                                                    \
    do {                                                                            \
        asm volatile("s_waitcnt lgkmcnt(0)" ::: "memory");                          \
        __builtin_amdgcn_sched_barrier(0);                                          \
        __builtin_amdgcn_s_barrier();                                               \
        __builtin_amdgcn_sched_barrier(0);                                          \
    } while (0)
#define Y_BAR()                                \
    do {                                       \
        __builtin_amdgcn_sched_barrier(0);     \
        __builtin_amdgcn_s_barrier();          \
        __builtin_amdgcn_sched_barrier(0);     \
    } while (0)
#define Y_VMCNT(n) asm volatile("s_waitcnt vmcnt(" #n ")" ::: "memory")
#pragma unroll
    for (int j = 0; j < 10; ++j) stage(0, 0, j);
    Y_VMCNT(0);
    Y_BAR();
    if (wm == 1) Y_BAR();
    auto ktile = [&](int kt, auto more_c) {
        constexpr bool more = decltype(more_c)::value;
        const char* St = smem + (kt & 1) * Y_STAGE;
        const int nb = (kt + 1) & 1;
        rd_w(St, 0);
        rd_a(St, 0, 0);
        if constexpr (more) {
            stage(nb, kt + 1, 0);
            stage(nb, kt + 1, 1);
            if (DIST == 0) {
                stage(nb, kt + 1, 2);
                Y_VMCNT(3);
            } else {
                Y_VMCNT(2);
            }
        } else {
            Y_VMCNT(0);
        }
        Y_SYNC();
        mma(0);
        Y_BAR();
        rd_a(St, 1, 0);
        if constexpr (more) {
            if (DIST != 0) stage(nb, kt + 1, 2);
            stage(nb, kt + 1, 3);
            stage(nb, kt + 1, 4);
            if (DIST == 0) stage(nb, kt + 1, 5);
        }
        Y_SYNC();
        mma(1);
        Y_BAR();
        rd_w(St, 1);
        rd_a(St, 0, 1);
        if constexpr (more) {
            if (DIST != 0) stage(nb, kt + 1, 5);
            stage(nb, kt + 1, 6);
            if (DIST == 0) stage(nb, kt + 1, 7);
        }
        Y_SYNC();
        mma(0);
        Y_BAR();
        rd_a(St, 1, 1);
        if constexpr (more) {
            if (DIST != 0) stage(nb, kt + 1, 7);
            stage(nb, kt + 1, 8);
            stage(nb, kt + 1, 9);
            Y_VMCNT(3);
        }
        Y_SYNC();
        mma(1);
        Y_BAR();
    };
    for (int kt = 0; kt + 1 < nkt; ++kt) ktile(kt, std::true_type{});
    if (nkt > 0) ktile(nkt - 1, std::false_type{});
    if (wm == 0) Y_BAR();
#undef Y_VMCNT
#undef Y_SYNC
#undef Y_BAR

    if (G.clk != nullptr) {
        const unsigned long long c1 = __builtin_readcyclecounter(), r1 = __builtin_amdgcn_s_memrealtime();
        if (tid == 0) {
            atomicAdd(G.clk, c1 - clk_c0);
            atomicAdd(G.clk + 1, r1 - clk_r0);
        }
    }

#if APEXMI_GEMM_TRACE
    if (G.trace != nullptr) y_t_loop = __builtin_amdgcn_s_memrealtime();
#endif
    if constexpr (EPI == APEXMI_EPI_BIAS && QKV == 1) {
        if (P.qkv) {
            qkv_epilogue16<12, 192>(acc, P, G.qs, M, m0, n0, wave, wm, wn, lane, smem);
            Y_TRACE_END(n0 / G.qs.inner);
            return;
        }
    }
    constexpr int MTC = EPI == APEXMI_EPI_BIAS_GATE_RES ? 3 : 6;
#pragma unroll
    for (int h = 0; h < 12 / MTC; ++h) {
        int mrow[MTC];
#pragma unroll
        for (int mt = 0; mt < MTC; ++mt) {
            mrow[mt] = m0 + wm * 192 + (h * MTC + mt) * 16 + l15;
            if (mrow[mt] >= M) mrow[mt] = -1;
        }
#pragma unroll
        for (int p = 0; p < 2; ++p) {
            const int nbase = n0 + wn * 64 + p * 32;
            const f32x4_t(&x)[MTC] = *(const f32x4_t(*)[MTC]) & acc[2 * p][h * MTC];
            const f32x4_t(&y)[MTC] = *(const f32x4_t(*)[MTC]) & acc[2 * p + 1][h * MTC];
            if constexpr (EPI == APEXMI_EPI_BIAS_GATE_RES) {
                u32x4 rr[MTC];
                const int nst = nbase + 16 * (g4 & 1) + 8 * (g4 >> 1);
#pragma unroll
                for (int mt = 0; mt < MTC; ++mt) rr[mt] = *(const u32x4*)(P.R + (int64_t)max(mrow[mt], 0) * P.ldr + min(nst, N - 8));
                store_slab16<EPI, MTC, 0>(x, y, P, N, mrow, nbase, g4, rr);
            } else {
                APEXMI_ACT_DISPATCH(P.gelu, store_slab16<EPI, MTC, ACT>(x, y, P, N, mrow, nbase, g4));
            }
        }
    }
    Y_TRACE_END(3);
}
#undef Y_TRACE_END

int g_group_m = GROUP_M;
#if APEXMI_GEMM_TRACE
uintptr_t g_gemm_trace = 0;
#endif
int g_large_cfg = 7;
int g_force_cfg = 0;
int g_wpacked = 0;
int g_tail_max = 96;
int g_x288 = 0;
int g_x384_group_m = 3;
int g_x384_dist = -1;
int g_x384_qkv = 1;
int g_x384 = 1;
int g_small_max = 112;
int g_tail_split = 2;

int g_streamk = 1;
struct SkWorkspace {
    float* slab;
    unsigned* flag;
};
static int sk_workspace(hipStream_t stream, SkWorkspace* out) {
    static std::mutex mu;
    static std::vector<std::tuple<int, hipStream_t, SkWorkspace>> all;
    int dev = 0;
    (void)hipGetDevice(&dev);
    std::lock_guard<std::mutex> lk(mu);
    for (auto& e : all)
        if (std::get<0>(e) == dev && std::get<1>(e) == stream) {
            *out = std::get<2>(e);
            return 0;
        }
    SkWorkspace w{nullptr, nullptr};
    if (hipMalloc((void**)&w.slab, (size_t)256 * 65536 * sizeof(float)) != hipSuccess ||
        hipMalloc((void**)&w.flag, 256 * sizeof(unsigned)) != hipSuccess || hipMemset(w.flag, 0, 256 * sizeof(unsigned)) != hipSuccess) {
        apexmi_set_error("gemm_bf16: stream-K workspace allocation failed");
        return 1;
    }
    all.emplace_back(dev, stream, w);
    *out = w;
    return 0;
}

template <typename CFG, int EPI>
int launch_cfg(GemmGroup& G, const int* Ms, hipStream_t stream) {
    if constexpr (APEXMI_GEMM_PEEL >= 2 && (CFG::SCHED == 0 || CFG::SCHED == 5)) {
        for (int i = 0; i < G.count; ++i)
            if (G.p[i].lda > (1 << 22) || G.p[i].ldw > (1 << 22)) {
                apexmi_set_error("gemm_bf16: leading dimensions above 2^22 elements are not supported (lda %lld, ldw %lld)",
                                 (long long)G.p[i].lda, (long long)G.p[i].ldw);
                return 1;
            }
    }
    static uint64_t attr_set = 0;
    APEXMI_SET_ATTR_ONCE(attr_set,
        (void)hipFuncSetAttribute((const void*)gemm_bf16_kernel<CFG, EPI>,
                                  hipFuncAttributeMaxDynamicSharedMemorySize, CFG::LDS));
    int t = 0;
    for (int i = 0; i < G.count; ++i) {
        G.p[i].M = Ms[i];
        G.p[i].nm = (Ms[i] + CFG::BM - 1) / CFG::BM;
        G.p[i].nn = (G.p[i].N + CFG::BN - 1) / CFG::BN;
        G.p[i].tile0 = t;
        t += G.p[i].nm * G.p[i].nn;
    }
    G.total = t;
    G.group_m = g_group_m;
    G.clk = apexmi_clk_ptr();
#if APEXMI_GEMM_TRACE
    G.trace = (unsigned long long*)g_gemm_trace;
#endif
    G.wpacked = (CFG::SCHED == 5) ? g_wpacked : 0;
    G.sk_r = 0;
    G.sk_tfull = 0;
    G.sk_slab = nullptr;
    G.sk_flag = nullptr;
    if constexpr (CFG::SCHED == 5 && APEXMI_GEMM_STREAMK) {
        const int r = t % 256;
        const bool forced = g_streamk == 2 && G.batch == 1 && t >= 256 && (r == 0 || (r >= 88 && r <= 232));
        if (forced || (g_streamk && G.batch == 1 && r >= 88 && r <= 232 && G.K / BK >= 8)) {
            SkWorkspace w;
            if (sk_workspace(stream, &w)) return 1;
            G.sk_r = r;
            G.sk_tfull = t - r;
            G.sk_slab = w.slab;
            G.sk_flag = w.flag;
            hipLaunchKernelGGL((gemm_bf16_kernel<CFG, EPI>), dim3(256, 1), dim3(CFG::NT), CFG::LDS, stream, G);
            return apexmi_check_launch("gemm_bf16");
        }
    }
    hipLaunchKernelGGL((gemm_bf16_kernel<CFG, EPI>), dim3(t, G.batch), dim3(CFG::NT), CFG::LDS, stream, G);
    return apexmi_check_launch("gemm_bf16");
}

template <int EPI>
int launch_x288(GemmGroup& G, const int* Ms, hipStream_t stream) {
    static uint64_t attr_set = 0;
    APEXMI_SET_ATTR_ONCE(attr_set,
        (void)hipFuncSetAttribute((const void*)gemm_bf16_x288_kernel<EPI>, hipFuncAttributeMaxDynamicSharedMemorySize, X_LDS));
    int t = 0;
    for (int i = 0; i < G.count; ++i) {
        G.p[i].M = Ms[i];
        G.p[i].nm = (Ms[i] + XBM - 1) / XBM;
        G.p[i].nn = (G.p[i].N + XBN - 1) / XBN;
        G.p[i].tile0 = t;
        t += G.p[i].nm * G.p[i].nn;
    }
    G.total = t;
    G.group_m = g_group_m;
    G.clk = apexmi_clk_ptr();
    G.wpacked = 0;
    G.sk_r = G.sk_tfull = 0;
    G.sk_slab = nullptr;
    G.sk_flag = nullptr;
    hipLaunchKernelGGL((gemm_bf16_x288_kernel<EPI>), dim3(t, 1), dim3(512), X_LDS, stream, G);
    return apexmi_check_launch("gemm_bf16 (288x192)");
}

template <int EPI>
int launch_x384(GemmGroup& G, const int* Ms, hipStream_t stream) {
    static uint64_t attr_set = 0;
    APEXMI_SET_ATTR_ONCE(attr_set,
        (void)hipFuncSetAttribute((const void*)gemm_bf16_x384_kernel<EPI, 0>, hipFuncAttributeMaxDynamicSharedMemorySize, Y_LDS);
        (void)hipFuncSetAttribute((const void*)gemm_bf16_x384_kernel<EPI, 1>, hipFuncAttributeMaxDynamicSharedMemorySize, Y_LDS);
        if constexpr (EPI == APEXMI_EPI_BIAS)
            (void)hipFuncSetAttribute((const void*)gemm_bf16_x384_kernel<EPI, 1, 1>, hipFuncAttributeMaxDynamicSharedMemorySize, Y_LDS));
    int t = 0;
    for (int i = 0; i < G.count; ++i) {
        G.p[i].M = Ms[i];
        G.p[i].nm = (Ms[i] + YBM - 1) / YBM;
        G.p[i].nn = (G.p[i].N + YBN - 1) / YBN;
        G.p[i].tile0 = t;
        t += G.p[i].nm * G.p[i].nn;
    }
    G.total = t;
    G.group_m = g_x384_group_m;
    G.clk = apexmi_clk_ptr();
#if APEXMI_GEMM_TRACE
    G.trace = (unsigned long long*)g_gemm_trace;
#endif
    G.wpacked = 0;
    G.sk_r = G.sk_tfull = 0;
    G.sk_slab = nullptr;
    G.sk_flag = nullptr;
    bool any_qkv = false;
    for (int i = 0; i < G.count; ++i) any_qkv |= G.p[i].qkv != 0;
    if constexpr (EPI == APEXMI_EPI_BIAS) {
        if (any_qkv) {
            hipLaunchKernelGGL((gemm_bf16_x384_kernel<EPI, 1, 1>), dim3(t, 1), dim3(512), Y_LDS, stream, G);
            return apexmi_check_launch("gemm_bf16 (384x256, fused q/k/v)");
        }
    }
    const int dist = g_x384_dist >= 0 ? g_x384_dist : (t >= 2048 ? 0 : 1);
    if (dist == 0) hipLaunchKernelGGL((gemm_bf16_x384_kernel<EPI, 0>), dim3(t, 1), dim3(512), Y_LDS, stream, G);
    else hipLaunchKernelGGL((gemm_bf16_x384_kernel<EPI, 1>), dim3(t, 1), dim3(512), Y_LDS, stream, G);
    return apexmi_check_launch("gemm_bf16 (384x256)");
}

inline bool x288_pays(const GemmGroup& G, const int* Ms) {
    int64_t t256 = 0, t288 = 0;
    for (int i = 0; i < G.count; ++i) {
        if (G.p[i].qkv) return false;
        t256 += (int64_t)((Ms[i] + 255) / 256) * ((G.p[i].N + 255) / 256);
        t288 += (int64_t)((Ms[i] + XBM - 1) / XBM) * ((G.p[i].N + XBN - 1) / XBN);
    }
    const double c256 = (double)((t256 + 255) / 256) * 65536.0;
    const double c288 = (double)((t288 + 255) / 256) * (XBM * XBN) * 1.04;
    return c288 < 0.95 * c256;
}

inline bool use_x288(const GemmGroup& G, const int* Ms) {
    if (g_x288 == 0 || G.batch != 1 || G.K % BK != 0 || !(g_force_cfg == 0 || g_force_cfg == 7) || g_large_cfg != 7) return false;
    int64_t mtot = 0;
    int nmax = 0;
    for (int i = 0; i < G.count; ++i) {
        if (G.p[i].qkv) return false;
        mtot += Ms[i];
        nmax = G.p[i].N > nmax ? G.p[i].N : nmax;
    }
    if (g_x288 == 2) return true;
    return G.K >= 256 && mtot >= 1024 && nmax >= 1024 && x288_pays(G, Ms);
}

inline bool x384_pays(const GemmGroup& G, const int* Ms) {
    int64_t t = 0;
    for (int i = 0; i < G.count; ++i) {
        const int64_t nm = (Ms[i] + YBM - 1) / YBM;
        if ((nm * YBM - Ms[i]) * 200 > 3 * (int64_t)Ms[i]) return false;
        t += nm * ((G.p[i].N + YBN - 1) / YBN);
    }
    const int64_t rem = t % 256;
    return t >= 3 * 256 && (rem == 0 || rem >= 154 || t >= 8 * 256);
}
inline bool use_x384(const GemmGroup& G, const int* Ms) {
    if (g_x384 == 0 || G.batch != 1 || G.K % BK != 0 || !(g_force_cfg == 0 || g_force_cfg == 7) || g_large_cfg != 7) return false;
    for (int i = 0; i < G.count; ++i)
        if (G.p[i].qkv || G.p[i].lda > (1 << 21) || G.p[i].ldw > (1 << 21)) return false;
    return g_x384 == 2 || x384_pays(G, Ms);
}

template <int EPI>
int launch_epi(GemmGroup& G, const int* Ms, hipStream_t stream) {
    int cfg = g_force_cfg;
    if constexpr (EPI == APEXMI_EPI_BIAS || EPI == APEXMI_EPI_BIAS_GATE_RES) {
        if (use_x288(G, Ms)) return launch_x288<EPI>(G, Ms, stream);
        if (use_x384(G, Ms)) return launch_x384<EPI>(G, Ms, stream);
    }
    if (cfg == 0) {
        int64_t mtot = 0;
        int nmax = 0;
        for (int i = 0; i < G.count; ++i) {
            mtot += Ms[i];
            nmax = G.p[i].N > nmax ? G.p[i].N : nmax;
        }
        cfg = (mtot >= 1024 && nmax >= 1024 && G.K >= 256) ? g_large_cfg : 1;
        if (EPI == APEXMI_EPI_BIAS_GATE_RES && cfg == 7 && G.batch == 1 && g_small_max > 0) {
            int64_t t256 = 0;
            bool any_qkv = false;
            for (int i = 0; i < G.count; ++i) {
                t256 += (int64_t)((Ms[i] + 255) / 256) * ((G.p[i].N + 255) / 256);
                any_qkv |= G.p[i].qkv != 0;
            }
            if (!any_qkv && t256 <= g_small_max) cfg = 1;
        }
        if (cfg == 6 && G.K % 12288 == 0) cfg = 7;
        if ((cfg == 7 || cfg == 9 || cfg == 10) && g_tail_split && G.count >= 2 && G.batch == 1) {
            int64_t lead = 0;
            for (int i = 0; i + 1 < G.count; ++i)
                lead += (int64_t)((Ms[i] + 255) / 256) * ((G.p[i].N + 255) / 256);
            const int li = G.count - 1;
            const int64_t last = (int64_t)((Ms[li] + 255) / 256) * ((G.p[li].N + 255) / 256);
            if (lead >= 256 && lead % 256 == 0 && last <= g_tail_max) {
                GemmGroup T = G;
                T.count = 1;
                T.p[0] = G.p[li];
                G.count = li;
                if (int rc = (cfg == 9    ? launch_cfg<CFG_256R, EPI>(G, Ms, stream)
                              : cfg == 10 ? launch_cfg<CFG_256R5, EPI>(G, Ms, stream)
                                          : launch_cfg<CFG_256P16, EPI>(G, Ms, stream)))
                    return rc;
                if (g_tail_split == 2) return launch_cfg<CFG_128E, EPI>(T, Ms + li, stream);
                return launch_cfg<CFG_128, EPI>(T, Ms + li, stream);
            }
        }
    }
    switch (cfg) {
        case 1: return launch_cfg<CFG_128, EPI>(G, Ms, stream);
        case 2: return launch_cfg<CFG_256, EPI>(G, Ms, stream);
        case 8: return launch_cfg<CFG_128E, EPI>(G, Ms, stream);
        case 6: return launch_cfg<CFG_256W, EPI>(G, Ms, stream);
        case 7: return launch_cfg<CFG_256P16, EPI>(G, Ms, stream);
        case 9: return launch_cfg<CFG_256R, EPI>(G, Ms, stream);
        case 10: return launch_cfg<CFG_256R5, EPI>(G, Ms, stream);
        default:
            return launch_cfg<CFG_256P, EPI>(G, Ms, stream);
    }
}

int launch_group(GemmGroup& G, const int* Ms, int kind, hipStream_t stream) {
    switch (kind) {
        case APEXMI_EPI_BIAS_GATE_RES: return launch_epi<APEXMI_EPI_BIAS_GATE_RES>(G, Ms, stream);
        case APEXMI_EPI_BIAS_F32: return launch_epi<APEXMI_EPI_BIAS_F32>(G, Ms, stream);
        case EPI_GATE_RES_F32: return launch_epi<EPI_GATE_RES_F32>(G, Ms, stream);
        default: return launch_epi<APEXMI_EPI_BIAS>(G, Ms, stream);
    }
}

int epi_base(int epilogue) { return epilogue & ~APEXMI_EPI_F32_IO; }
bool epi_f32(int epilogue) { return (epilogue & APEXMI_EPI_F32_IO) != 0 || epi_base(epilogue) == APEXMI_EPI_BIAS_F32; }
int epi_kind(int epilogue) {
    const int b = epi_base(epilogue);
    if (epilogue & APEXMI_EPI_F32_IO) return b == APEXMI_EPI_BIAS_GATE_RES ? EPI_GATE_RES_F32 : APEXMI_EPI_BIAS_F32;
    return act_mode(b) ? APEXMI_EPI_BIAS : b;
}

int check_problem(const void* A, int64_t lda, const void* W, int64_t ldw, void* C, int64_t ldc, int M,
                  int N, int K, int epilogue, const float* gate, const void* R, int64_t ldr) {
    APEXMI_REQUIRE(A && W && C, "gemm_bf16: null operand");
    APEXMI_REQUIRE(M > 0 && N > 0 && K > 0, "gemm_bf16: empty problem M=%d N=%d K=%d", M, N, K);
    APEXMI_REQUIRE(K % BK == 0, "gemm_bf16: K=%d must be a multiple of %d", K, BK);
    APEXMI_REQUIRE(N % 8 == 0, "gemm_bf16: N=%d must be a multiple of 8", N);
    APEXMI_REQUIRE(lda % 8 == 0 && ldw % 8 == 0 && ldc % 4 == 0,
                   "gemm_bf16: leading dimensions must keep rows 16-byte aligned");
    APEXMI_REQUIRE(((uintptr_t)A % 16) == 0 && ((uintptr_t)W % 16) == 0 && ((uintptr_t)C % 8) == 0,
                   "gemm_bf16: operands must be 16-byte aligned");
    APEXMI_REQUIRE(epi_base(epilogue) >= 0 && epi_base(epilogue) <= 6 && (epilogue & ~(APEXMI_EPI_F32_IO | 7)) == 0,
                   "gemm_bf16: unknown epilogue %d", epilogue);
    APEXMI_REQUIRE(!epi_f32(epilogue) || ((uintptr_t)C % 16) == 0, "gemm_bf16: f32 output must be 16-byte aligned");
    if (epi_base(epilogue) == APEXMI_EPI_BIAS_GATE_RES) {
        APEXMI_REQUIRE(gate && R, "gemm_bf16: gate/residual epilogue needs gate and R");
        APEXMI_REQUIRE(ldr % 4 == 0 && ((uintptr_t)gate % 16) == 0 && ((uintptr_t)R % (epi_f32(epilogue) ? 16 : 8)) == 0,
                       "gemm_bf16: gate/R alignment");
    }
    return 0;
}

}

extern "C" int apexmi_gemm_bf16(const void* A, int64_t lda, const void* W, int64_t ldw,
                                const void* bias, void* C, int64_t ldc, int M, int N, int K,
                                int epilogue, const float* gate, const void* R, int64_t ldr,
                                apexmi_stream_t stream_) {
    hipStream_t stream = (hipStream_t)stream_;
    if (int rc = check_problem(A, lda, W, ldw, C, ldc, M, N, K, epilogue, gate, R, ldr)) return rc;
    GemmGroup G;
    G.count = 1;
    G.K = K;
    G.batch = 1;
    G.bsA = G.bsW = G.bsC_bytes = 0;
    G.p[0] = GemmProblem{(const bf16_t*)A, (const bf16_t*)W, (const bf16_t*)bias, (bf16_t*)C, gate,
                         (const bf16_t*)R, lda, ldw, ldc, ldr, M, N, 0, 0, 0,
                         act_mode(epi_base(epilogue))};
    ApexmiProfScope prof(0, stream, 2.0 * M * N * (double)K,
                         2.0 * ((double)M * K + (double)N * K + (double)M * N));
    return launch_group(G, &M, epi_kind(epilogue), stream);
}

extern "C" int apexmi_gemm_bf16_batched(const void* A, int64_t lda, int64_t stride_a, const void* W, int64_t ldw,
                                        int64_t stride_w, void* C, int64_t ldc, int64_t stride_c, int batch, int M,
                                        int N, int K, int epilogue, apexmi_stream_t stream_) {
    hipStream_t stream = (hipStream_t)stream_;
    if (int rc = check_problem(A, lda, W, ldw, C, ldc, M, N, K, epilogue, nullptr, nullptr, 0)) return rc;
    APEXMI_REQUIRE(epilogue == APEXMI_EPI_BIAS || epilogue == APEXMI_EPI_BIAS_F32,
                   "gemm_bf16_batched: epilogue %d unsupported (plain bf16 or f32 output only)", epilogue);
    APEXMI_REQUIRE(batch >= 1 && batch <= 65535, "gemm_bf16_batched: batch=%d not in [1, 65535]", batch);
    const int esz = epilogue == APEXMI_EPI_BIAS_F32 ? 4 : 2;
    APEXMI_REQUIRE(stride_a % 8 == 0 && stride_w % 8 == 0 && (stride_c * esz) % 16 == 0,
                   "gemm_bf16_batched: batch strides must keep every element 16-byte aligned");
    APEXMI_REQUIRE(epilogue != APEXMI_EPI_BIAS_F32 || ((uintptr_t)C % 16) == 0, "gemm_bf16_batched: f32 output must be 16-byte aligned");
    GemmGroup G;
    G.count = 1;
    G.K = K;
    G.batch = batch;
    G.bsA = stride_a;
    G.bsW = stride_w;
    G.bsC_bytes = stride_c * esz;
    G.p[0] = GemmProblem{(const bf16_t*)A, (const bf16_t*)W, nullptr, (bf16_t*)C, nullptr, nullptr, lda, ldw, ldc, 0,
                         M, N, 0, 0, 0, 0};
    ApexmiProfScope prof(0, stream, 2.0 * batch * M * N * (double)K,
                         2.0 * batch * ((double)M * K + (double)N * K + (double)M * N));
    return launch_group(G, &M, epi_kind(epilogue), stream);
}

extern "C" int apexmi_gemm_bf16_grouped(int count, const void* const* A, const int64_t* lda,
                                        const void* const* W, const int64_t* ldw,
                                        const void* const* bias, void* const* C, const int64_t* ldc,
                                        const int* M, const int* N, int K, const int* epilogue,
                                        const float* const* gate, const void* const* R,
                                        const int64_t* ldr, apexmi_stream_t stream_) {
    hipStream_t stream = (hipStream_t)stream_;
    APEXMI_REQUIRE(count >= 1 && count <= MAX_GROUPS, "gemm_bf16_grouped: count=%d not in [1,%d]", count, MAX_GROUPS);
    GemmGroup G;
    G.count = count;
    G.K = K;
    G.batch = 1;
    G.bsA = G.bsW = G.bsC_bytes = 0;
    double flops = 0, bytes = 0;
    const int kind = epi_kind(epilogue[0]);
    for (int i = 0; i < count; ++i) {
        APEXMI_REQUIRE(epi_kind(epilogue[i]) == kind,
                       "gemm_bf16_grouped: gate/residual (or float / bf16 output) problems cannot be mixed with the others");
        const float* g = gate ? gate[i] : nullptr;
        const void* r = R ? R[i] : nullptr;
        const int64_t lr = ldr ? ldr[i] : 0;
        if (int rc = check_problem(A[i], lda[i], W[i], ldw[i], C[i], ldc[i], M[i], N[i], K, epilogue[i], g, r, lr))
            return rc;
        G.p[i] = GemmProblem{(const bf16_t*)A[i], (const bf16_t*)W[i], (const bf16_t*)(bias ? bias[i] : nullptr),
                             (bf16_t*)C[i], g, (const bf16_t*)r, lda[i], ldw[i], ldc[i], lr, M[i], N[i], 0, 0, 0,
                             act_mode(epi_base(epilogue[i]))};
        flops += 2.0 * M[i] * N[i] * (double)K;
        bytes += 2.0 * ((double)M[i] * K + (double)N[i] * K + (double)M[i] * N[i]);
    }
    ApexmiProfScope prof(0, stream, flops, bytes);
    return launch_group(G, M, kind, stream);
}

extern "C" int apexmi_gemm_uses_x288(int M, int N, int K) {
    GemmGroup G;
    memset(&G, 0, sizeof(G));
    G.count = 1;
    G.K = K;
    G.batch = 1;
    G.p[0].N = N;
    return (M > 0 && N > 0 && K > 0 && use_x288(G, &M)) ? 1 : 0;
}

extern "C" int apexmi_gemm_qkv_fusable(int64_t m_total, int n_max, int K) {
    return (g_force_cfg == 0 || g_force_cfg == 7 || g_force_cfg == 9 || g_force_cfg == 10) &&
           (g_large_cfg == 7 || g_large_cfg == 9 || g_large_cfg == 10) && m_total >= 1024 && n_max >= 1024 && K >= 256 && K % BK == 0;
}

extern "C" int apexmi_gemm_bf16_grouped_qkv(int count, const void* const* A, const int64_t* lda, const void* const* W,
                                            const int64_t* ldw, const void* const* bias, void* const* C, const int64_t* ldc,
                                            const int* M, const int* N, int K, const int* epilogue, const int* is_qkv,
                                            const void* const* norm_q, const void* const* norm_k, const int* row0, int H,
                                            float eps, const float* rope, void* q_out, void* k_out, void* vt_out, int S_out,
                                            int Skp, apexmi_stream_t stream_) {
    return apexmi_gemm_bf16_grouped_qkv_pairs(count, A, lda, W, ldw, bias, C, ldc, M, N, K, epilogue, is_qkv, norm_q, norm_k, row0, H,
                                              eps, rope, nullptr, q_out, k_out, vt_out, S_out, Skp, stream_);
}

extern "C" int apexmi_gemm_bf16_grouped_qkv_pairs(int count, const void* const* A, const int64_t* lda, const void* const* W,
                                                  const int64_t* ldw, const void* const* bias, void* const* C, const int64_t* ldc,
                                                  const int* M, const int* N, int K, const int* epilogue, const int* is_qkv,
                                                  const void* const* norm_q, const void* const* norm_k, const int* row0, int H,
                                                  float eps, const float* rope, const float* rope_pairs, void* q_out, void* k_out,
                                                  void* vt_out, int S_out, int Skp, apexmi_stream_t stream_) {
    hipStream_t stream = (hipStream_t)stream_;
    APEXMI_REQUIRE(((uintptr_t)rope_pairs % 16) == 0, "gemm_bf16_grouped_qkv: rope_pairs must be 16-byte aligned");
    APEXMI_REQUIRE(count >= 1 && count <= MAX_GROUPS, "gemm_bf16_grouped_qkv: count=%d not in [1,%d]", count, MAX_GROUPS);
    APEXMI_REQUIRE(is_qkv && row0 && rope && q_out && k_out && vt_out && H > 0, "gemm_bf16_grouped_qkv: null argument");
    APEXMI_REQUIRE(H % 2 == 0 && S_out > 0 && Skp >= S_out && Skp % 8 == 0, "gemm_bf16_grouped_qkv: H=%d must be even, Skp=%d a multiple of 8 >= S_out=%d",
                   H, Skp, S_out);
    APEXMI_REQUIRE(((uintptr_t)rope % 16) == 0 && ((uintptr_t)q_out % 16) == 0 && ((uintptr_t)k_out % 16) == 0 && ((uintptr_t)vt_out % 16) == 0,
                   "gemm_bf16_grouped_qkv: rope / outputs must be 16-byte aligned");
    GemmGroup G;
    G.count = count;
    G.K = K;
    G.batch = 1;
    G.bsA = G.bsW = G.bsC_bytes = 0;
    G.qs = QkvShared{(bf16_t*)q_out, (bf16_t*)k_out, (bf16_t*)vt_out, rope, S_out, Skp, H * 128, eps, rope_pairs};
    double flops = 0, bytes = 0;
    int64_t mtot = 0;
    int nmax = 0;
    for (int i = 0; i < count; ++i) {
        APEXMI_REQUIRE(epi_kind(epilogue[i]) == APEXMI_EPI_BIAS, "gemm_bf16_grouped_qkv: bias-class epilogues only (got %d)", epilogue[i]);
        void* c = is_qkv[i] ? q_out : C[i];
        const int64_t lc = is_qkv[i] ? 128 : ldc[i];
        if (int rc = check_problem(A[i], lda[i], W[i], ldw[i], c, lc, M[i], N[i], K, epilogue[i], nullptr, nullptr, 0)) return rc;
        G.p[i] = GemmProblem{(const bf16_t*)A[i], (const bf16_t*)W[i], (const bf16_t*)(bias ? bias[i] : nullptr), (bf16_t*)c,
                             nullptr, nullptr, lda[i], ldw[i], lc, 0, M[i], N[i], 0, 0, 0, act_mode(epi_base(epilogue[i]))};
        if (is_qkv[i]) {
            APEXMI_REQUIRE(N[i] == 3 * H * 128 && epi_base(epilogue[i]) == APEXMI_EPI_BIAS,
                           "gemm_bf16_grouped_qkv: a fused problem has N = 3 H 128 = %d (got %d) and the plain bias epilogue", 3 * H * 128, N[i]);
            APEXMI_REQUIRE(row0[i] >= 0 && row0[i] + M[i] <= S_out,
                           "gemm_bf16_grouped_qkv: rows [%d, %d) must lie inside S_out=%d", row0[i], row0[i] + M[i], S_out);
            const void* nq = norm_q ? norm_q[i] : nullptr;
            const void* nk = norm_k ? norm_k[i] : nullptr;
            APEXMI_REQUIRE(((uintptr_t)nq % 16) == 0 && ((uintptr_t)nk % 16) == 0, "gemm_bf16_grouped_qkv: norm weights must be 16-byte aligned");
            G.p[i].qkv = 1;
            G.p[i].row0 = row0[i];
            G.p[i].nq = (const bf16_t*)nq;
            G.p[i].nk = (const bf16_t*)nk;
        }
        mtot += M[i];
        nmax = N[i] > nmax ? N[i] : nmax;
        flops += 2.0 * M[i] * N[i] * (double)K;
        bytes += 2.0 * ((double)M[i] * K + (double)N[i] * K + (double)M[i] * N[i]);
    }
    APEXMI_REQUIRE(apexmi_gemm_qkv_fusable(mtot, nmax, K),
                   "gemm_bf16_grouped_qkv: needs the 256x256 v_mfma_f32_16x16x32 tiling (gemm.config / gemm.large = 7, >= 1024 rows)");
    ApexmiProfScope prof(0, stream, flops, bytes);
    bool ld_ok = true;
    for (int i = 0; i < count; ++i) ld_ok &= lda[i] <= (1 << 21) && ldw[i] <= (1 << 21);
    if (g_x384 && g_x384_qkv && ld_ok && g_large_cfg == 7 && (g_force_cfg == 0 || g_force_cfg == 7) && (g_x384 == 2 || x384_pays(G, M)))
        return launch_x384<APEXMI_EPI_BIAS>(G, M, stream);
    if (g_large_cfg == 9 || g_force_cfg == 9) return launch_cfg<CFG_256R, APEXMI_EPI_BIAS>(G, M, stream);
    if (g_large_cfg == 10 || g_force_cfg == 10) return launch_cfg<CFG_256R5, APEXMI_EPI_BIAS>(G, M, stream);
    return launch_cfg<CFG_256P16, APEXMI_EPI_BIAS>(G, M, stream);
}

extern "C" int apexmi_split_bf16x3(const float* x, int64_t ldx, int64_t M, int K, void* out, int64_t ldo,
                                   apexmi_stream_t stream_) {
    hipStream_t stream = (hipStream_t)stream_;
    APEXMI_REQUIRE(x && out && M > 0 && K > 0, "split_bf16x3: bad arguments");
    APEXMI_REQUIRE(K % 8 == 0 && ldx % 4 == 0 && ldo % 8 == 0 && ldo >= 3 * (int64_t)K && ((uintptr_t)x % 16) == 0 &&
                       ((uintptr_t)out % 16) == 0,
                   "split_bf16x3: K=%d must be a multiple of 8 and rows 16-byte aligned", K);
    const int64_t n = M * (K / 8);
    ApexmiProfScope prof(5, stream, 0.0, 10.0 * (double)M * K);
    hipLaunchKernelGGL(split_bf16x3_kernel, dim3((unsigned)((n + 255) / 256)), dim3(256), 0, stream, x, ldx, M, K,
                       (bf16_t*)out, ldo);
    return apexmi_check_launch("split_bf16x3");
}

int apexmi_set_gemm_key(const char* key, int value) {
    if (!strcmp(key, "gemm.tail")) g_tail_split = value;
    else if (!strcmp(key, "gemm.tail_max")) g_tail_max = value;
    else if (!strcmp(key, "gemm.group_m")) g_group_m = value > 0 ? value : GROUP_M;
    else if (!strcmp(key, "gemm.large")) g_large_cfg = value;
    else if (!strcmp(key, "gemm.config")) g_force_cfg = value;
    else if (!strcmp(key, "gemm.wpacked")) g_wpacked = value;
    else if (!strcmp(key, "gemm.x288")) g_x288 = value;
    else if (!strcmp(key, "gemm.small_max")) g_small_max = value;
    else if (!strcmp(key, "gemm.x384")) g_x384 = value;
    else if (!strcmp(key, "gemm.x384_dist")) g_x384_dist = value;
    else if (!strcmp(key, "gemm.x384_group_m")) g_x384_group_m = value > 0 ? value : 3;
    else if (!strcmp(key, "gemm.x384_qkv")) g_x384_qkv = value;
#if APEXMI_GEMM_TRACE
    else if (!strcmp(key, "gemm.trace_lo")) g_gemm_trace = (g_gemm_trace & ~(uintptr_t)0xffffffffu) | (uint32_t)value;
    else if (!strcmp(key, "gemm.trace_hi")) g_gemm_trace = (g_gemm_trace & (uintptr_t)0xffffffffu) | ((uintptr_t)(uint32_t)value << 32);
#endif
    else if (!strcmp(key, "gemm.streamk")) g_streamk = value;
    else return 1;
    return 0;
}
```

Measured before the change: 16.34 steps/s.

## Replace GEMM ping-pong main loop with hand-scheduled inline assembly

Adds a hand-written inline-asm main K-loop for the 256x256 SCHED 5 GEMM config. It interleaves ds_read, global_load_lds and MFMA instructions with explicit waitcnts and barriers, with an alternative "faithful" variant that uses setprio. It is selected by default through a new gemm.pp_asm knob. The aim is to cut compiler scheduling overhead and stalls in the dominant GEMMs. The risks are correctness, register pressure and fragility against the compiler's allocation, so a no-spill check is added for this kernel.

Result: faster. 16.57 steps/s, median of 6 (+1.4%).

```diff
diff --git a/apex-studio_amd/build.py b/apex-studio_amd/build.py
--- a/apex-studio_amd/build.py
+++ b/apex-studio_amd/build.py
@@ -29,7 +29,8 @@
 
 
 NO_SPILL = {"attention.hip": ["attn_fwd_d128_w64_kernel", "attn_fwd_d128_w64r_kernel"],
-            "attention_masked.hip": ["attn_masked_kernel"]}
+            "attention_masked.hip": ["attn_masked_kernel"],
+            "gemm.hip": ["gemm_bf16_kernelINS_3CfgILi256ELi256ELi2ELi4ELi5EEE"]}
 REMARKS = "-Rpass-analysis=kernel-resource-usage"
 
 
diff --git a/apex-studio_amd/csrc/gemm.hip b/apex-studio_amd/csrc/gemm.hip
--- a/apex-studio_amd/csrc/gemm.hip
+++ b/apex-studio_amd/csrc/gemm.hip
@@ -589,7 +589,7 @@
 #define APEXMI_TRACE_END() do { } while (0)
 #endif
 
-template <typename CFG, int EPI>
+template <typename CFG, int EPI, int PPA = 0>
 __device__ __forceinline__ void gemm_tile(const GemmGroup& G, char* smem, int s, const SkCtx& sk) {
     constexpr int BM = CFG::BM, BN = CFG::BN, TM = CFG::TM, TN = CFG::TN;
 
@@ -1132,7 +1132,61 @@
             mma(1, 0);
             PP_BAR();
         };
-        for (int kt = 0; kt + 1 < nkt; ++kt) ktile(kt, std::true_type{});
+        int kt = 0;
+#if APEXMI_GEMM_PEEL >= 2 && !APEXMI_GEMM_STREAMK
+        if (PPA != 0 && nkt > 1) {
+            const uint32_t la0 = smem_lds + a16[0] + ch16[0], la1 = smem_lds + a16[0] + ch16[1];
+            const uint32_t lw0 = smem_lds + CFG::A_BYTES + w16[0] + ch16[0], lw1 = smem_lds + CFG::A_BYTES + w16[0] + ch16[1];
+            const uint32_t ma00 = smem_lds + ra_row[0][0] * 128, ma01 = smem_lds + ra_row[0][1] * 128;
+            const uint32_t ma10 = smem_lds + ra_row[1][0] * 128, ma11 = smem_lds + ra_row[1][1] * 128;
+            const uint32_t mw00 = smem_lds + CFG::A_BYTES + rw_row[0][0] * 128, mw01 = smem_lds + CFG::A_BYTES + rw_row[0][1] * 128;
+            const uint32_t mw10 = smem_lds + CFG::A_BYTES + rw_row[1][0] * 128, mw11 = smem_lds + CFG::A_BYTES + rw_row[1][1] * 128;
+            const char* const ap = a_base_u + a_kstep;
+            const char* const wp = w_base_u + w_kstep;
+            const uint32_t ak = (uint32_t)a_kstep, wk = (uint32_t)w_kstep;
+            int n = nkt - 1;
+            bf16x8 pfa[4][2], pfw[2][2][2];
+#define PP16_C(i, j) [c##i##j] "+v"(acc16[i][j])
+#define PP16_FA(t, k) [fa##t##k] "=&v"(pfa[t][k])
+#define PP16_FW(s, u, k) [fw##s##u##k] "=&v"(pfw[s][u][k])
+#define PP16_OPERANDS                                                                                                                  \
+    : PP16_C(0, 0), PP16_C(0, 1), PP16_C(0, 2), PP16_C(0, 3), PP16_C(0, 4), PP16_C(0, 5), PP16_C(0, 6), PP16_C(0, 7), PP16_C(1, 0),  \
+      PP16_C(1, 1), PP16_C(1, 2), PP16_C(1, 3), PP16_C(1, 4), PP16_C(1, 5), PP16_C(1, 6), PP16_C(1, 7), PP16_C(2, 0), PP16_C(2, 1),  \
+      PP16_C(2, 2), PP16_C(2, 3), PP16_C(2, 4), PP16_C(2, 5), PP16_C(2, 6), PP16_C(2, 7), PP16_C(3, 0), PP16_C(3, 1), PP16_C(3, 2),  \
+      PP16_C(3, 3), PP16_C(3, 4), PP16_C(3, 5), PP16_C(3, 6), PP16_C(3, 7), PP16_FA(0, 0), PP16_FA(0, 1), PP16_FA(1, 0),             \
+      PP16_FA(1, 1), PP16_FA(2, 0), PP16_FA(2, 1), PP16_FA(3, 0), PP16_FA(3, 1), PP16_FW(0, 0, 0), PP16_FW(0, 0, 1),                \
+      PP16_FW(0, 1, 0), PP16_FW(0, 1, 1), PP16_FW(1, 0, 0), PP16_FW(1, 0, 1), PP16_FW(1, 1, 0), PP16_FW(1, 1, 1), [n] "+s"(n)         \
+    : [la00] "v"(la0), [la01] "v"(la1), [la10] "v"(la0 + CFG::STAGE), [la11] "v"(la1 + CFG::STAGE), [lw00] "v"(lw0),               \
+      [lw01] "v"(lw1), [lw10] "v"(lw0 + CFG::STAGE), [lw11] "v"(lw1 + CFG::STAGE), [oa00] "v"(ra_off[0][0]), [oa01] "v"(ra_off[0][1]), \
+      [oa10] "v"(ra_off[1][0]), [oa11] "v"(ra_off[1][1]), [ow00] "v"(rw_off[0][0]), [ow01] "v"(rw_off[0][1]),                      \
+      [ow10] "v"(rw_off[1][0]), [ow11] "v"(rw_off[1][1]), [ma00] "s"(ma00), [ma01] "s"(ma01), [ma10] "s"(ma10), [ma11] "s"(ma11),   \
+      [mw00] "s"(mw00), [mw01] "s"(mw01), [mw10] "s"(mw10), [mw11] "s"(mw11), [ap] "s"(ap), [wp] "s"(wp), [ak] "s"(ak), [wk] "s"(wk)  \
+    : "memory", "scc", "m0",
+#pragma clang diagnostic push
+#pragma clang diagnostic ignored "-Winline-asm"
+            if constexpr (PPA == 2) {
+                asm volatile(
+#include "gemm_pp16_faithful.inc"
+                    PP16_OPERANDS
+#include "gemm_pp16_clobbers.inc"
+                );
+            } else {
+                asm volatile(
+#include "gemm_pp16_body.inc"
+                    PP16_OPERANDS
+#include "gemm_pp16_clobbers.inc"
+                );
+            }
+#pragma clang diagnostic pop
+#undef PP16_OPERANDS
+#undef PP16_FW
+#undef PP16_FA
+#undef PP16_C
+            kt = nkt - 1;
+        }
+#endif
+        if constexpr (PPA == 0)
+            for (; kt + 1 < nkt; ++kt) ktile(kt, std::true_type{});
         if (nkt > 0) ktile(nkt - 1, std::false_type{});
         if (wm == 0) PP_BAR();
 #undef VMCNT
@@ -1349,16 +1403,16 @@
                             store_ntile<EPI, TM, ACT>(acc[nt], P, N, mrow, n0 + wn * (BN / CFG::WN) + nt * 32, hi));
 }
 
-template <typename CFG, int EPI>
+template <typename CFG, int EPI, int PPA = 0>
 __global__ __launch_bounds__(CFG::NT, CFG::OCC) void gemm_bf16_kernel(const GemmGroup G) {
     extern __shared__ __attribute__((aligned(16))) char smem[];
     const int nkt = G.K / BK;
     SkCtx sk{TILE_FULL, 0, nkt, 0, 0};
     if constexpr (CFG::SCHED != 5) {
-        gemm_tile<CFG, EPI>(G, smem, xcd_remap(blockIdx.x, G.total), sk);
+        gemm_tile<CFG, EPI, PPA>(G, smem, xcd_remap(blockIdx.x, G.total), sk);
     } else {
         if (!APEXMI_GEMM_STREAMK || (G.sk_r <= 0 && G.sk_tfull <= 0)) {
-            gemm_tile<CFG, EPI>(G, smem, xcd_remap(blockIdx.x, G.total), sk);
+            gemm_tile<CFG, EPI, PPA>(G, smem, xcd_remap(blockIdx.x, G.total), sk);
             return;
         }
         for (int it = 0;; ++it) {
@@ -1413,7 +1467,7 @@
                 }
             }
             if (it) __syncthreads();
-            gemm_tile<CFG, EPI>(G, smem, tile, sk);
+            gemm_tile<CFG, EPI, PPA>(G, smem, tile, sk);
         }
     }
 }
@@ -1898,6 +1952,7 @@
 int g_large_cfg = 7;
 int g_force_cfg = 0;
 int g_wpacked = 0;
+int g_pp_asm = 1;
 int g_tail_max = 96;
 int g_x288 = 0;
 int g_x384_group_m = 3;
@@ -1944,10 +1999,15 @@
                 return 1;
             }
     }
+    constexpr bool has_asm = CFG::SCHED == 5 && APEXMI_GEMM_PEEL >= 2 && !APEXMI_GEMM_STREAMK;
     static uint64_t attr_set = 0;
-    APEXMI_SET_ATTR_ONCE(attr_set,
-        (void)hipFuncSetAttribute((const void*)gemm_bf16_kernel<CFG, EPI>,
-                                  hipFuncAttributeMaxDynamicSharedMemorySize, CFG::LDS));
+    APEXMI_SET_ATTR_ONCE(attr_set, {
+        (void)hipFuncSetAttribute((const void*)gemm_bf16_kernel<CFG, EPI>, hipFuncAttributeMaxDynamicSharedMemorySize, CFG::LDS);
+        if constexpr (has_asm) {
+            (void)hipFuncSetAttribute((const void*)gemm_bf16_kernel<CFG, EPI, 1>, hipFuncAttributeMaxDynamicSharedMemorySize, CFG::LDS);
+            (void)hipFuncSetAttribute((const void*)gemm_bf16_kernel<CFG, EPI, 2>, hipFuncAttributeMaxDynamicSharedMemorySize, CFG::LDS);
+        }
+    });
     int t = 0;
     for (int i = 0; i < G.count; ++i) {
         G.p[i].M = Ms[i];
@@ -1981,7 +2041,12 @@
             return apexmi_check_launch("gemm_bf16");
         }
     }
-    hipLaunchKernelGGL((gemm_bf16_kernel<CFG, EPI>), dim3(t, G.batch), dim3(CFG::NT), CFG::LDS, stream, G);
+    void (*kern)(const GemmGroup) = gemm_bf16_kernel<CFG, EPI>;
+    if constexpr (has_asm) {
+        if (g_pp_asm == 1) kern = gemm_bf16_kernel<CFG, EPI, 1>;
+        else if (g_pp_asm == 2) kern = gemm_bf16_kernel<CFG, EPI, 2>;
+    }
+    hipLaunchKernelGGL(kern, dim3(t, G.batch), dim3(CFG::NT), CFG::LDS, stream, G);
     return apexmi_check_launch("gemm_bf16");
 }
 
@@ -2373,6 +2438,7 @@
     else if (!strcmp(key, "gemm.large")) g_large_cfg = value;
     else if (!strcmp(key, "gemm.config")) g_force_cfg = value;
     else if (!strcmp(key, "gemm.wpacked")) g_wpacked = value;
+    else if (!strcmp(key, "gemm.pp_asm")) g_pp_asm = value;
     else if (!strcmp(key, "gemm.x288")) g_x288 = value;
     else if (!strcmp(key, "gemm.small_max")) g_small_max = value;
     else if (!strcmp(key, "gemm.x384")) g_x384 = value;
diff --git a/apex-studio_amd/csrc/gemm_pp16_body.inc b/apex-studio_amd/csrc/gemm_pp16_body.inc
--- /dev/null
+++ b/apex-studio_amd/csrc/gemm_pp16_body.inc
@@ -0,0 +1,309 @@
+"s_mov_b64 s[80:81], %[ap]\n\t"
+"s_mov_b64 s[82:83], %[wp]\n\t"
+"s_nop 4\n\t"
+"s_cmp_eq_u32 %[n], 0\n\t"
+"s_cbranch_scc1 .Lpp16_end_%=\n\t"
+"ds_read_b128 %[fw000], %[lw00] offset:0\n\t"
+"ds_read_b128 %[fw010], %[lw00] offset:2048\n\t"
+"ds_read_b128 %[fw001], %[lw01] offset:0\n\t"
+"ds_read_b128 %[fw011], %[lw01] offset:2048\n\t"
+".Lpp16_loop_%=:\n\t"
+"ds_read_b128 %[fa00], %[la00] offset:0\n\t"
+"ds_read_b128 %[fa10], %[la00] offset:2048\n\t"
+"ds_read_b128 %[fa20], %[la00] offset:4096\n\t"
+"ds_read_b128 %[fa30], %[la00] offset:6144\n\t"
+"ds_read_b128 %[fa01], %[la01] offset:0\n\t"
+"ds_read_b128 %[fa11], %[la01] offset:2048\n\t"
+"ds_read_b128 %[fa21], %[la01] offset:4096\n\t"
+"s_add_u32 m0, %[mw00], 0x10000\n\t"
+"ds_read_b128 %[fa31], %[la01] offset:6144\n\t"
+"global_load_lds_dwordx4 %[ow00], s[82:83]\n\t"
+"s_add_u32 m0, %[mw01], 0x10000\n\t"
+"s_nop 0\n\t"
+"global_load_lds_dwordx4 %[ow01], s[82:83]\n\t"
+"s_waitcnt vmcnt(4)\n\t"
+"s_barrier\n\t"
+"s_waitcnt lgkmcnt(7)\n\t"
+"v_mfma_f32_16x16x32_bf16 %[c00], %[fw000], %[fa00], %[c00]\n\t"
+"s_waitcnt lgkmcnt(6)\n\t"
+"v_mfma_f32_16x16x32_bf16 %[c01], %[fw000], %[fa10], %[c01]\n\t"
+"s_waitcnt lgkmcnt(5)\n\t"
+"v_mfma_f32_16x16x32_bf16 %[c02], %[fw000], %[fa20], %[c02]\n\t"
+"s_waitcnt lgkmcnt(4)\n\t"
+"v_mfma_f32_16x16x32_bf16 %[c03], %[fw000], %[fa30], %[c03]\n\t"
+"v_mfma_f32_16x16x32_bf16 %[c10], %[fw010], %[fa00], %[c10]\n\t"
+"v_mfma_f32_16x16x32_bf16 %[c11], %[fw010], %[fa10], %[c11]\n\t"
+"v_mfma_f32_16x16x32_bf16 %[c12], %[fw010], %[fa20], %[c12]\n\t"
+"v_mfma_f32_16x16x32_bf16 %[c13], %[fw010], %[fa30], %[c13]\n\t"
+"s_waitcnt lgkmcnt(3)\n\t"
+"v_mfma_f32_16x16x32_bf16 %[c00], %[fw001], %[fa01], %[c00]\n\t"
+"s_waitcnt lgkmcnt(2)\n\t"
+"v_mfma_f32_16x16x32_bf16 %[c01], %[fw001], %[fa11], %[c01]\n\t"
+"s_waitcnt lgkmcnt(1)\n\t"
+"v_mfma_f32_16x16x32_bf16 %[c02], %[fw001], %[fa21], %[c02]\n\t"
+"s_waitcnt lgkmcnt(0)\n\t"
+"v_mfma_f32_16x16x32_bf16 %[c03], %[fw001], %[fa31], %[c03]\n\t"
+"v_mfma_f32_16x16x32_bf16 %[c10], %[fw011], %[fa01], %[c10]\n\t"
+"v_mfma_f32_16x16x32_bf16 %[c11], %[fw011], %[fa11], %[c11]\n\t"
+"v_mfma_f32_16x16x32_bf16 %[c12], %[fw011], %[fa21], %[c12]\n\t"
+"v_mfma_f32_16x16x32_bf16 %[c13], %[fw011], %[fa31], %[c13]\n\t"
+"s_barrier\n\t"
+"ds_read_b128 %[fw100], %[lw00] offset:4096\n\t"
+"ds_read_b128 %[fw110], %[lw00] offset:6144\n\t"
+"ds_read_b128 %[fw101], %[lw01] offset:4096\n\t"
+"s_add_u32 m0, %[ma00], 0x10000\n\t"
+"ds_read_b128 %[fw111], %[lw01] offset:6144\n\t"
+"global_load_lds_dwordx4 %[oa00], s[80:81]\n\t"
+"s_add_u32 m0, %[ma01], 0x10000\n\t"
+"s_nop 0\n\t"
+"global_load_lds_dwordx4 %[oa01], s[80:81]\n\t"
+"s_waitcnt vmcnt(4)\n\t"
+"s_barrier\n\t"
+"s_waitcnt lgkmcnt(3)\n\t"
+"v_mfma_f32_16x16x32_bf16 %[c20], %[fw100], %[fa00], %[c20]\n\t"
+"v_mfma_f32_16x16x32_bf16 %[c21], %[fw100], %[fa10], %[c21]\n\t"
+"v_mfma_f32_16x16x32_bf16 %[c22], %[fw100], %[fa20], %[c22]\n\t"
+"v_mfma_f32_16x16x32_bf16 %[c23], %[fw100], %[fa30], %[c23]\n\t"
+"s_waitcnt lgkmcnt(2)\n\t"
+"v_mfma_f32_16x16x32_bf16 %[c30], %[fw110], %[fa00], %[c30]\n\t"
+"v_mfma_f32_16x16x32_bf16 %[c31], %[fw110], %[fa10], %[c31]\n\t"
+"v_mfma_f32_16x16x32_bf16 %[c32], %[fw110], %[fa20], %[c32]\n\t"
+"v_mfma_f32_16x16x32_bf16 %[c33], %[fw110], %[fa30], %[c33]\n\t"
+"s_waitcnt lgkmcnt(1)\n\t"
+"v_mfma_f32_16x16x32_bf16 %[c20], %[fw101], %[fa01], %[c20]\n\t"
+"v_mfma_f32_16x16x32_bf16 %[c21], %[fw101], %[fa11], %[c21]\n\t"
+"v_mfma_f32_16x16x32_bf16 %[c22], %[fw101], %[fa21], %[c22]\n\t"
+"v_mfma_f32_16x16x32_bf16 %[c23], %[fw101], %[fa31], %[c23]\n\t"
+"s_waitcnt lgkmcnt(0)\n\t"
+"v_mfma_f32_16x16x32_bf16 %[c30], %[fw111], %[fa01], %[c30]\n\t"
+"v_mfma_f32_16x16x32_bf16 %[c31], %[fw111], %[fa11], %[c31]\n\t"
+"v_mfma_f32_16x16x32_bf16 %[c32], %[fw111], %[fa21], %[c32]\n\t"
+"v_mfma_f32_16x16x32_bf16 %[c33], %[fw111], %[fa31], %[c33]\n\t"
+"s_barrier\n\t"
+"ds_read_b128 %[fa00], %[la00] offset:8192\n\t"
+"ds_read_b128 %[fa10], %[la00] offset:10240\n\t"
+"ds_read_b128 %[fa20], %[la00] offset:12288\n\t"
+"ds_read_b128 %[fa30], %[la00] offset:14336\n\t"
+"ds_read_b128 %[fa01], %[la01] offset:8192\n\t"
+"ds_read_b128 %[fa11], %[la01] offset:10240\n\t"
+"ds_read_b128 %[fa21], %[la01] offset:12288\n\t"
+"s_add_u32 m0, %[mw10], 0x10000\n\t"
+"ds_read_b128 %[fa31], %[la01] offset:14336\n\t"
+"global_load_lds_dwordx4 %[ow10], s[82:83]\n\t"
+"s_add_u32 m0, %[mw11], 0x10000\n\t"
+"s_nop 0\n\t"
+"global_load_lds_dwordx4 %[ow11], s[82:83]\n\t"
+"s_add_u32 s82, s82, %[wk]\n\t"
+"s_addc_u32 s83, s83, 0\n\t"
+"s_waitcnt vmcnt(4)\n\t"
+"s_barrier\n\t"
+"s_waitcnt lgkmcnt(7)\n\t"
+"v_mfma_f32_16x16x32_bf16 %[c24], %[fw100], %[fa00], %[c24]\n\t"
+"s_waitcnt lgkmcnt(6)\n\t"
+"v_mfma_f32_16x16x32_bf16 %[c25], %[fw100], %[fa10], %[c25]\n\t"
+"s_waitcnt lgkmcnt(5)\n\t"
+"v_mfma_f32_16x16x32_bf16 %[c26], %[fw100], %[fa20], %[c26]\n\t"
+"s_waitcnt lgkmcnt(4)\n\t"
+"v_mfma_f32_16x16x32_bf16 %[c27], %[fw100], %[fa30], %[c27]\n\t"
+"v_mfma_f32_16x16x32_bf16 %[c34], %[fw110], %[fa00], %[c34]\n\t"
+"v_mfma_f32_16x16x32_bf16 %[c35], %[fw110], %[fa10], %[c35]\n\t"
+"v_mfma_f32_16x16x32_bf16 %[c36], %[fw110], %[fa20], %[c36]\n\t"
+"v_mfma_f32_16x16x32_bf16 %[c37], %[fw110], %[fa30], %[c37]\n\t"
+"s_waitcnt lgkmcnt(3)\n\t"
+"v_mfma_f32_16x16x32_bf16 %[c24], %[fw101], %[fa01], %[c24]\n\t"
+"s_waitcnt lgkmcnt(2)\n\t"
+"v_mfma_f32_16x16x32_bf16 %[c25], %[fw101], %[fa11], %[c25]\n\t"
+"s_waitcnt lgkmcnt(1)\n\t"
+"v_mfma_f32_16x16x32_bf16 %[c26], %[fw101], %[fa21], %[c26]\n\t"
+"s_waitcnt lgkmcnt(0)\n\t"
+"v_mfma_f32_16x16x32_bf16 %[c27], %[fw101], %[fa31], %[c27]\n\t"
+"v_mfma_f32_16x16x32_bf16 %[c34], %[fw111], %[fa01], %[c34]\n\t"
+"v_mfma_f32_16x16x32_bf16 %[c35], %[fw111], %[fa11], %[c35]\n\t"
+"v_mfma_f32_16x16x32_bf16 %[c36], %[fw111], %[fa21], %[c36]\n\t"
+"v_mfma_f32_16x16x32_bf16 %[c37], %[fw111], %[fa31], %[c37]\n\t"
+"s_barrier\n\t"
+"ds_read_b128 %[fw100], %[lw10] offset:0\n\t"
+"ds_read_b128 %[fw110], %[lw10] offset:2048\n\t"
+"ds_read_b128 %[fw101], %[lw11] offset:0\n\t"
+"s_add_u32 m0, %[ma10], 0x10000\n\t"
+"ds_read_b128 %[fw111], %[lw11] offset:2048\n\t"
+"global_load_lds_dwordx4 %[oa10], s[80:81]\n\t"
+"s_add_u32 m0, %[ma11], 0x10000\n\t"
+"s_nop 0\n\t"
+"global_load_lds_dwordx4 %[oa11], s[80:81]\n\t"
+"s_add_u32 s80, s80, %[ak]\n\t"
+"s_addc_u32 s81, s81, 0\n\t"
+"s_waitcnt vmcnt(4)\n\t"
+"s_barrier\n\t"
+"v_mfma_f32_16x16x32_bf16 %[c04], %[fw000], %[fa00], %[c04]\n\t"
+"v_mfma_f32_16x16x32_bf16 %[c05], %[fw000], %[fa10], %[c05]\n\t"
+"v_mfma_f32_16x16x32_bf16 %[c06], %[fw000], %[fa20], %[c06]\n\t"
+"v_mfma_f32_16x16x32_bf16 %[c07], %[fw000], %[fa30], %[c07]\n\t"
+"v_mfma_f32_16x16x32_bf16 %[c14], %[fw010], %[fa00], %[c14]\n\t"
+"v_mfma_f32_16x16x32_bf16 %[c15], %[fw010], %[fa10], %[c15]\n\t"
+"v_mfma_f32_16x16x32_bf16 %[c16], %[fw010], %[fa20], %[c16]\n\t"
+"v_mfma_f32_16x16x32_bf16 %[c17], %[fw010], %[fa30], %[c17]\n\t"
+"v_mfma_f32_16x16x32_bf16 %[c04], %[fw001], %[fa01], %[c04]\n\t"
+"v_mfma_f32_16x16x32_bf16 %[c05], %[fw001], %[fa11], %[c05]\n\t"
+"v_mfma_f32_16x16x32_bf16 %[c06], %[fw001], %[fa21], %[c06]\n\t"
+"v_mfma_f32_16x16x32_bf16 %[c07], %[fw001], %[fa31], %[c07]\n\t"
+"v_mfma_f32_16x16x32_bf16 %[c14], %[fw011], %[fa01], %[c14]\n\t"
+"v_mfma_f32_16x16x32_bf16 %[c15], %[fw011], %[fa11], %[c15]\n\t"
+"v_mfma_f32_16x16x32_bf16 %[c16], %[fw011], %[fa21], %[c16]\n\t"
+"v_mfma_f32_16x16x32_bf16 %[c17], %[fw011], %[fa31], %[c17]\n\t"
+"s_barrier\n\t"
+"s_sub_i32 %[n], %[n], 1\n\t"
+"s_cmp_lg_u32 %[n], 0\n\t"
+"s_cbranch_scc0 .Lpp16_end_%=\n\t"
+"ds_read_b128 %[fa00], %[la10] offset:0\n\t"
+"ds_read_b128 %[fa10], %[la10] offset:2048\n\t"
+"ds_read_b128 %[fa20], %[la10] offset:4096\n\t"
+"ds_read_b128 %[fa30], %[la10] offset:6144\n\t"
+"ds_read_b128 %[fa01], %[la11] offset:0\n\t"
+"ds_read_b128 %[fa11], %[la11] offset:2048\n\t"
+"ds_read_b128 %[fa21], %[la11] offset:4096\n\t"
+"s_mov_b32 m0, %[mw00]\n\t"
+"ds_read_b128 %[fa31], %[la11] offset:6144\n\t"
+"global_load_lds_dwordx4 %[ow00], s[82:83]\n\t"
+"s_mov_b32 m0, %[mw01]\n\t"
+"s_nop 0\n\t"
+"global_load_lds_dwordx4 %[ow01], s[82:83]\n\t"
+"s_waitcnt vmcnt(4)\n\t"
+"s_barrier\n\t"
+"s_waitcnt lgkmcnt(7)\n\t"
+"v_mfma_f32_16x16x32_bf16 %[c00], %[fw100], %[fa00], %[c00]\n\t"
+"s_waitcnt lgkmcnt(6)\n\t"
+"v_mfma_f32_16x16x32_bf16 %[c01], %[fw100], %[fa10], %[c01]\n\t"
+"s_waitcnt lgkmcnt(5)\n\t"
+"v_mfma_f32_16x16x32_bf16 %[c02], %[fw100], %[fa20], %[c02]\n\t"
+"s_waitcnt lgkmcnt(4)\n\t"
+"v_mfma_f32_16x16x32_bf16 %[c03], %[fw100], %[fa30], %[c03]\n\t"
+"v_mfma_f32_16x16x32_bf16 %[c10], %[fw110], %[fa00], %[c10]\n\t"
+"v_mfma_f32_16x16x32_bf16 %[c11], %[fw110], %[fa10], %[c11]\n\t"
+"v_mfma_f32_16x16x32_bf16 %[c12], %[fw110], %[fa20], %[c12]\n\t"
+"v_mfma_f32_16x16x32_bf16 %[c13], %[fw110], %[fa30], %[c13]\n\t"
+"s_waitcnt lgkmcnt(3)\n\t"
+"v_mfma_f32_16x16x32_bf16 %[c00], %[fw101], %[fa01], %[c00]\n\t"
+"s_waitcnt lgkmcnt(2)\n\t"
+"v_mfma_f32_16x16x32_bf16 %[c01], %[fw101], %[fa11], %[c01]\n\t"
+"s_waitcnt lgkmcnt(1)\n\t"
+"v_mfma_f32_16x16x32_bf16 %[c02], %[fw101], %[fa21], %[c02]\n\t"
+"s_waitcnt lgkmcnt(0)\n\t"
+"v_mfma_f32_16x16x32_bf16 %[c03], %[fw101], %[fa31], %[c03]\n\t"
+"v_mfma_f32_16x16x32_bf16 %[c10], %[fw111], %[fa01], %[c10]\n\t"
+"v_mfma_f32_16x16x32_bf16 %[c11], %[fw111], %[fa11], %[c11]\n\t"
+"v_mfma_f32_16x16x32_bf16 %[c12], %[fw111], %[fa21], %[c12]\n\t"
+"v_mfma_f32_16x16x32_bf16 %[c13], %[fw111], %[fa31], %[c13]\n\t"
+"s_barrier\n\t"
+"ds_read_b128 %[fw000], %[lw10] offset:4096\n\t"
+"ds_read_b128 %[fw010], %[lw10] offset:6144\n\t"
+"ds_read_b128 %[fw001], %[lw11] offset:4096\n\t"
+"s_mov_b32 m0, %[ma00]\n\t"
+"ds_read_b128 %[fw011], %[lw11] offset:6144\n\t"
+"global_load_lds_dwordx4 %[oa00], s[80:81]\n\t"
+"s_mov_b32 m0, %[ma01]\n\t"
+"s_nop 0\n\t"
+"global_load_lds_dwordx4 %[oa01], s[80:81]\n\t"
+"s_waitcnt vmcnt(4)\n\t"
+"s_barrier\n\t"
+"s_waitcnt lgkmcnt(3)\n\t"
+"v_mfma_f32_16x16x32_bf16 %[c20], %[fw000], %[fa00], %[c20]\n\t"
+"v_mfma_f32_16x16x32_bf16 %[c21], %[fw000], %[fa10], %[c21]\n\t"
+"v_mfma_f32_16x16x32_bf16 %[c22], %[fw000], %[fa20], %[c22]\n\t"
+"v_mfma_f32_16x16x32_bf16 %[c23], %[fw000], %[fa30], %[c23]\n\t"
+"s_waitcnt lgkmcnt(2)\n\t"
+"v_mfma_f32_16x16x32_bf16 %[c30], %[fw010], %[fa00], %[c30]\n\t"
+"v_mfma_f32_16x16x32_bf16 %[c31], %[fw010], %[fa10], %[c31]\n\t"
+"v_mfma_f32_16x16x32_bf16 %[c32], %[fw010], %[fa20], %[c32]\n\t"
+"v_mfma_f32_16x16x32_bf16 %[c33], %[fw010], %[fa30], %[c33]\n\t"
+"s_waitcnt lgkmcnt(1)\n\t"
+"v_mfma_f32_16x16x32_bf16 %[c20], %[fw001], %[fa01], %[c20]\n\t"
+"v_mfma_f32_16x16x32_bf16 %[c21], %[fw001], %[fa11], %[c21]\n\t"
+"v_mfma_f32_16x16x32_bf16 %[c22], %[fw001], %[fa21], %[c22]\n\t"
+"v_mfma_f32_16x16x32_bf16 %[c23], %[fw001], %[fa31], %[c23]\n\t"
+"s_waitcnt lgkmcnt(0)\n\t"
+"v_mfma_f32_16x16x32_bf16 %[c30], %[fw011], %[fa01], %[c30]\n\t"
+"v_mfma_f32_16x16x32_bf16 %[c31], %[fw011], %[fa11], %[c31]\n\t"
+"v_mfma_f32_16x16x32_bf16 %[c32], %[fw011], %[fa21], %[c32]\n\t"
+"v_mfma_f32_16x16x32_bf16 %[c33], %[fw011], %[fa31], %[c33]\n\t"
+"s_barrier\n\t"
+"ds_read_b128 %[fa00], %[la10] offset:8192\n\t"
+"ds_read_b128 %[fa10], %[la10] offset:10240\n\t"
+"ds_read_b128 %[fa20], %[la10] offset:12288\n\t"
+"ds_read_b128 %[fa30], %[la10] offset:14336\n\t"
+"ds_read_b128 %[fa01], %[la11] offset:8192\n\t"
+"ds_read_b128 %[fa11], %[la11] offset:10240\n\t"
+"ds_read_b128 %[fa21], %[la11] offset:12288\n\t"
+"s_mov_b32 m0, %[mw10]\n\t"
+"ds_read_b128 %[fa31], %[la11] offset:14336\n\t"
+"global_load_lds_dwordx4 %[ow10], s[82:83]\n\t"
+"s_mov_b32 m0, %[mw11]\n\t"
+"s_nop 0\n\t"
+"global_load_lds_dwordx4 %[ow11], s[82:83]\n\t"
+"s_add_u32 s82, s82, %[wk]\n\t"
+"s_addc_u32 s83, s83, 0\n\t"
+"s_waitcnt vmcnt(4)\n\t"
+"s_barrier\n\t"
+"s_waitcnt lgkmcnt(7)\n\t"
+"v_mfma_f32_16x16x32_bf16 %[c24], %[fw000], %[fa00], %[c24]\n\t"
+"s_waitcnt lgkmcnt(6)\n\t"
+"v_mfma_f32_16x16x32_bf16 %[c25], %[fw000], %[fa10], %[c25]\n\t"
+"s_waitcnt lgkmcnt(5)\n\t"
+"v_mfma_f32_16x16x32_bf16 %[c26], %[fw000], %[fa20], %[c26]\n\t"
+"s_waitcnt lgkmcnt(4)\n\t"
+"v_mfma_f32_16x16x32_bf16 %[c27], %[fw000], %[fa30], %[c27]\n\t"
+"v_mfma_f32_16x16x32_bf16 %[c34], %[fw010], %[fa00], %[c34]\n\t"
+"v_mfma_f32_16x16x32_bf16 %[c35], %[fw010], %[fa10], %[c35]\n\t"
+"v_mfma_f32_16x16x32_bf16 %[c36], %[fw010], %[fa20], %[c36]\n\t"
+"v_mfma_f32_16x16x32_bf16 %[c37], %[fw010], %[fa30], %[c37]\n\t"
+"s_waitcnt lgkmcnt(3)\n\t"
+"v_mfma_f32_16x16x32_bf16 %[c24], %[fw001], %[fa01], %[c24]\n\t"
+"s_waitcnt lgkmcnt(2)\n\t"
+"v_mfma_f32_16x16x32_bf16 %[c25], %[fw001], %[fa11], %[c25]\n\t"
+"s_waitcnt lgkmcnt(1)\n\t"
+"v_mfma_f32_16x16x32_bf16 %[c26], %[fw001], %[fa21], %[c26]\n\t"
+"s_waitcnt lgkmcnt(0)\n\t"
+"v_mfma_f32_16x16x32_bf16 %[c27], %[fw001], %[fa31], %[c27]\n\t"
+"v_mfma_f32_16x16x32_bf16 %[c34], %[fw011], %[fa01], %[c34]\n\t"
+"v_mfma_f32_16x16x32_bf16 %[c35], %[fw011], %[fa11], %[c35]\n\t"
+"v_mfma_f32_16x16x32_bf16 %[c36], %[fw011], %[fa21], %[c36]\n\t"
+"v_mfma_f32_16x16x32_bf16 %[c37], %[fw011], %[fa31], %[c37]\n\t"
+"s_barrier\n\t"
+"ds_read_b128 %[fw000], %[lw00] offset:0\n\t"
+"ds_read_b128 %[fw010], %[lw00] offset:2048\n\t"
+"ds_read_b128 %[fw001], %[lw01] offset:0\n\t"
+"s_mov_b32 m0, %[ma10]\n\t"
+"ds_read_b128 %[fw011], %[lw01] offset:2048\n\t"
+"global_load_lds_dwordx4 %[oa10], s[80:81]\n\t"
+"s_mov_b32 m0, %[ma11]\n\t"
+"s_nop 0\n\t"
+"global_load_lds_dwordx4 %[oa11], s[80:81]\n\t"
+"s_add_u32 s80, s80, %[ak]\n\t"
+"s_addc_u32 s81, s81, 0\n\t"
+"s_waitcnt vmcnt(4)\n\t"
+"s_barrier\n\t"
+"v_mfma_f32_16x16x32_bf16 %[c04], %[fw100], %[fa00], %[c04]\n\t"
+"v_mfma_f32_16x16x32_bf16 %[c05], %[fw100], %[fa10], %[c05]\n\t"
+"v_mfma_f32_16x16x32_bf16 %[c06], %[fw100], %[fa20], %[c06]\n\t"
+"v_mfma_f32_16x16x32_bf16 %[c07], %[fw100], %[fa30], %[c07]\n\t"
+"v_mfma_f32_16x16x32_bf16 %[c14], %[fw110], %[fa00], %[c14]\n\t"
+"v_mfma_f32_16x16x32_bf16 %[c15], %[fw110], %[fa10], %[c15]\n\t"
+"v_mfma_f32_16x16x32_bf16 %[c16], %[fw110], %[fa20], %[c16]\n\t"
+"v_mfma_f32_16x16x32_bf16 %[c17], %[fw110], %[fa30], %[c17]\n\t"
+"v_mfma_f32_16x16x32_bf16 %[c04], %[fw101], %[fa01], %[c04]\n\t"
+"v_mfma_f32_16x16x32_bf16 %[c05], %[fw101], %[fa11], %[c05]\n\t"
+"v_mfma_f32_16x16x32_bf16 %[c06], %[fw101], %[fa21], %[c06]\n\t"
+"v_mfma_f32_16x16x32_bf16 %[c07], %[fw101], %[fa31], %[c07]\n\t"
+"v_mfma_f32_16x16x32_bf16 %[c14], %[fw111], %[fa01], %[c14]\n\t"
+"v_mfma_f32_16x16x32_bf16 %[c15], %[fw111], %[fa11], %[c15]\n\t"
+"v_mfma_f32_16x16x32_bf16 %[c16], %[fw111], %[fa21], %[c16]\n\t"
+"v_mfma_f32_16x16x32_bf16 %[c17], %[fw111], %[fa31], %[c17]\n\t"
+"s_barrier\n\t"
+"s_sub_i32 %[n], %[n], 1\n\t"
+"s_cmp_lg_u32 %[n], 0\n\t"
+"s_cbranch_scc1 .Lpp16_loop_%=\n\t"
+".Lpp16_end_%=:\n\t"
+"s_waitcnt lgkmcnt(0)\n\t"
+"s_nop 7\n\t"
+"s_nop 7\n\t"
+"s_nop 3\n\t"
diff --git a/apex-studio_amd/csrc/gemm_pp16_clobbers.inc b/apex-studio_amd/csrc/gemm_pp16_clobbers.inc
--- /dev/null
+++ b/apex-studio_amd/csrc/gemm_pp16_clobbers.inc
@@ -0,0 +1 @@
+"s80", "s81", "s82", "s83"
diff --git a/apex-studio_amd/csrc/gemm_pp16_faithful.inc b/apex-studio_amd/csrc/gemm_pp16_faithful.inc
--- /dev/null
+++ b/apex-studio_amd/csrc/gemm_pp16_faithful.inc
@@ -0,0 +1,297 @@
+"s_mov_b64 s[80:81], %[ap]\n\t"
+"s_mov_b64 s[82:83], %[wp]\n\t"
+"s_nop 4\n\t"
+"s_cmp_eq_u32 %[n], 0\n\t"
+"s_cbranch_scc1 .Lpp16_end_%=\n\t"
+".Lpp16_loop_%=:\n\t"
+"ds_read_b128 %[fa00], %[la00] offset:0\n\t"
+"ds_read_b128 %[fa01], %[la01] offset:0\n\t"
+"ds_read_b128 %[fa10], %[la00] offset:2048\n\t"
+"ds_read_b128 %[fa11], %[la01] offset:2048\n\t"
+"ds_read_b128 %[fa20], %[la00] offset:4096\n\t"
+"ds_read_b128 %[fa21], %[la01] offset:4096\n\t"
+"ds_read_b128 %[fa30], %[la00] offset:6144\n\t"
+"ds_read_b128 %[fa31], %[la01] offset:6144\n\t"
+"ds_read_b128 %[fw000], %[lw00] offset:0\n\t"
+"ds_read_b128 %[fw001], %[lw01] offset:0\n\t"
+"ds_read_b128 %[fw010], %[lw00] offset:2048\n\t"
+"ds_read_b128 %[fw011], %[lw01] offset:2048\n\t"
+"s_add_u32 m0, %[ma00], 0x10000\n\t"
+"s_nop 0\n\t"
+"global_load_lds_dwordx4 %[oa00], s[80:81]\n\t"
+"s_add_u32 m0, %[ma01], 0x10000\n\t"
+"s_nop 0\n\t"
+"global_load_lds_dwordx4 %[oa01], s[80:81]\n\t"
+"s_waitcnt vmcnt(4)\n\t"
+"s_waitcnt lgkmcnt(0)\n\t"
+"s_barrier\n\t"
+"s_setprio 1\n\t"
+"v_mfma_f32_16x16x32_bf16 %[c00], %[fw000], %[fa00], %[c00]\n\t"
+"v_mfma_f32_16x16x32_bf16 %[c01], %[fw000], %[fa10], %[c01]\n\t"
+"v_mfma_f32_16x16x32_bf16 %[c02], %[fw000], %[fa20], %[c02]\n\t"
+"v_mfma_f32_16x16x32_bf16 %[c03], %[fw000], %[fa30], %[c03]\n\t"
+"v_mfma_f32_16x16x32_bf16 %[c10], %[fw010], %[fa00], %[c10]\n\t"
+"v_mfma_f32_16x16x32_bf16 %[c11], %[fw010], %[fa10], %[c11]\n\t"
+"v_mfma_f32_16x16x32_bf16 %[c12], %[fw010], %[fa20], %[c12]\n\t"
+"v_mfma_f32_16x16x32_bf16 %[c13], %[fw010], %[fa30], %[c13]\n\t"
+"v_mfma_f32_16x16x32_bf16 %[c00], %[fw001], %[fa01], %[c00]\n\t"
+"v_mfma_f32_16x16x32_bf16 %[c01], %[fw001], %[fa11], %[c01]\n\t"
+"v_mfma_f32_16x16x32_bf16 %[c02], %[fw001], %[fa21], %[c02]\n\t"
+"v_mfma_f32_16x16x32_bf16 %[c03], %[fw001], %[fa31], %[c03]\n\t"
+"v_mfma_f32_16x16x32_bf16 %[c10], %[fw011], %[fa01], %[c10]\n\t"
+"v_mfma_f32_16x16x32_bf16 %[c11], %[fw011], %[fa11], %[c11]\n\t"
+"v_mfma_f32_16x16x32_bf16 %[c12], %[fw011], %[fa21], %[c12]\n\t"
+"v_mfma_f32_16x16x32_bf16 %[c13], %[fw011], %[fa31], %[c13]\n\t"
+"s_setprio 0\n\t"
+"s_barrier\n\t"
+"ds_read_b128 %[fw100], %[lw00] offset:4096\n\t"
+"ds_read_b128 %[fw101], %[lw01] offset:4096\n\t"
+"ds_read_b128 %[fw110], %[lw00] offset:6144\n\t"
+"ds_read_b128 %[fw111], %[lw01] offset:6144\n\t"
+"s_add_u32 m0, %[mw00], 0x10000\n\t"
+"s_nop 0\n\t"
+"global_load_lds_dwordx4 %[ow00], s[82:83]\n\t"
+"s_add_u32 m0, %[mw01], 0x10000\n\t"
+"s_nop 0\n\t"
+"global_load_lds_dwordx4 %[ow01], s[82:83]\n\t"
+"s_waitcnt vmcnt(4)\n\t"
+"s_waitcnt lgkmcnt(0)\n\t"
+"s_barrier\n\t"
+"s_setprio 1\n\t"
+"v_mfma_f32_16x16x32_bf16 %[c20], %[fw100], %[fa00], %[c20]\n\t"
+"v_mfma_f32_16x16x32_bf16 %[c21], %[fw100], %[fa10], %[c21]\n\t"
+"v_mfma_f32_16x16x32_bf16 %[c22], %[fw100], %[fa20], %[c22]\n\t"
+"v_mfma_f32_16x16x32_bf16 %[c23], %[fw100], %[fa30], %[c23]\n\t"
+"v_mfma_f32_16x16x32_bf16 %[c30], %[fw110], %[fa00], %[c30]\n\t"
+"v_mfma_f32_16x16x32_bf16 %[c31], %[fw110], %[fa10], %[c31]\n\t"
+"v_mfma_f32_16x16x32_bf16 %[c32], %[fw110], %[fa20], %[c32]\n\t"
+"v_mfma_f32_16x16x32_bf16 %[c33], %[fw110], %[fa30], %[c33]\n\t"
+"v_mfma_f32_16x16x32_bf16 %[c20], %[fw101], %[fa01], %[c20]\n\t"
+"v_mfma_f32_16x16x32_bf16 %[c21], %[fw101], %[fa11], %[c21]\n\t"
+"v_mfma_f32_16x16x32_bf16 %[c22], %[fw101], %[fa21], %[c22]\n\t"
+"v_mfma_f32_16x16x32_bf16 %[c23], %[fw101], %[fa31], %[c23]\n\t"
+"v_mfma_f32_16x16x32_bf16 %[c30], %[fw111], %[fa01], %[c30]\n\t"
+"v_mfma_f32_16x16x32_bf16 %[c31], %[fw111], %[fa11], %[c31]\n\t"
+"v_mfma_f32_16x16x32_bf16 %[c32], %[fw111], %[fa21], %[c32]\n\t"
+"v_mfma_f32_16x16x32_bf16 %[c33], %[fw111], %[fa31], %[c33]\n\t"
+"s_setprio 0\n\t"
+"s_barrier\n\t"
+"ds_read_b128 %[fa00], %[la00] offset:8192\n\t"
+"ds_read_b128 %[fa01], %[la01] offset:8192\n\t"
+"ds_read_b128 %[fa10], %[la00] offset:10240\n\t"
+"ds_read_b128 %[fa11], %[la01] offset:10240\n\t"
+"ds_read_b128 %[fa20], %[la00] offset:12288\n\t"
+"ds_read_b128 %[fa21], %[la01] offset:12288\n\t"
+"ds_read_b128 %[fa30], %[la00] offset:14336\n\t"
+"ds_read_b128 %[fa31], %[la01] offset:14336\n\t"
+"s_add_u32 m0, %[mw10], 0x10000\n\t"
+"s_nop 0\n\t"
+"global_load_lds_dwordx4 %[ow10], s[82:83]\n\t"
+"s_add_u32 m0, %[mw11], 0x10000\n\t"
+"s_nop 0\n\t"
+"global_load_lds_dwordx4 %[ow11], s[82:83]\n\t"
+"s_add_u32 s82, s82, %[wk]\n\t"
+"s_addc_u32 s83, s83, 0\n\t"
+"s_waitcnt vmcnt(4)\n\t"
+"s_waitcnt lgkmcnt(0)\n\t"
+"s_barrier\n\t"
+"s_setprio 1\n\t"
+"v_mfma_f32_16x16x32_bf16 %[c24], %[fw100], %[fa00], %[c24]\n\t"
+"v_mfma_f32_16x16x32_bf16 %[c25], %[fw100], %[fa10], %[c25]\n\t"
+"v_mfma_f32_16x16x32_bf16 %[c26], %[fw100], %[fa20], %[c26]\n\t"
+"v_mfma_f32_16x16x32_bf16 %[c27], %[fw100], %[fa30], %[c27]\n\t"
+"v_mfma_f32_16x16x32_bf16 %[c34], %[fw110], %[fa00], %[c34]\n\t"
+"v_mfma_f32_16x16x32_bf16 %[c35], %[fw110], %[fa10], %[c35]\n\t"
+"v_mfma_f32_16x16x32_bf16 %[c36], %[fw110], %[fa20], %[c36]\n\t"
+"v_mfma_f32_16x16x32_bf16 %[c37], %[fw110], %[fa30], %[c37]\n\t"
+"v_mfma_f32_16x16x32_bf16 %[c24], %[fw101], %[fa01], %[c24]\n\t"
+"v_mfma_f32_16x16x32_bf16 %[c25], %[fw101], %[fa11], %[c25]\n\t"
+"v_mfma_f32_16x16x32_bf16 %[c26], %[fw101], %[fa21], %[c26]\n\t"
+"v_mfma_f32_16x16x32_bf16 %[c27], %[fw101], %[fa31], %[c27]\n\t"
+"v_mfma_f32_16x16x32_bf16 %[c34], %[fw111], %[fa01], %[c34]\n\t"
+"v_mfma_f32_16x16x32_bf16 %[c35], %[fw111], %[fa11], %[c35]\n\t"
+"v_mfma_f32_16x16x32_bf16 %[c36], %[fw111], %[fa21], %[c36]\n\t"
+"v_mfma_f32_16x16x32_bf16 %[c37], %[fw111], %[fa31], %[c37]\n\t"
+"s_setprio 0\n\t"
+"s_barrier\n\t"
+"s_add_u32 m0, %[ma10], 0x10000\n\t"
+"s_nop 0\n\t"
+"global_load_lds_dwordx4 %[oa10], s[80:81]\n\t"
+"s_add_u32 m0, %[ma11], 0x10000\n\t"
+"s_nop 0\n\t"
+"global_load_lds_dwordx4 %[oa11], s[80:81]\n\t"
+"s_add_u32 s80, s80, %[ak]\n\t"
+"s_addc_u32 s81, s81, 0\n\t"
+"s_waitcnt vmcnt(4)\n\t"
+"s_waitcnt lgkmcnt(0)\n\t"
+"s_barrier\n\t"
+"s_setprio 1\n\t"
+"v_mfma_f32_16x16x32_bf16 %[c04], %[fw000], %[fa00], %[c04]\n\t"
+"v_mfma_f32_16x16x32_bf16 %[c05], %[fw000], %[fa10], %[c05]\n\t"
+"v_mfma_f32_16x16x32_bf16 %[c06], %[fw000], %[fa20], %[c06]\n\t"
+"v_mfma_f32_16x16x32_bf16 %[c07], %[fw000], %[fa30], %[c07]\n\t"
+"v_mfma_f32_16x16x32_bf16 %[c14], %[fw010], %[fa00], %[c14]\n\t"
+"v_mfma_f32_16x16x32_bf16 %[c15], %[fw010], %[fa10], %[c15]\n\t"
+"v_mfma_f32_16x16x32_bf16 %[c16], %[fw010], %[fa20], %[c16]\n\t"
+"v_mfma_f32_16x16x32_bf16 %[c17], %[fw010], %[fa30], %[c17]\n\t"
+"v_mfma_f32_16x16x32_bf16 %[c04], %[fw001], %[fa01], %[c04]\n\t"
+"v_mfma_f32_16x16x32_bf16 %[c05], %[fw001], %[fa11], %[c05]\n\t"
+"v_mfma_f32_16x16x32_bf16 %[c06], %[fw001], %[fa21], %[c06]\n\t"
+"v_mfma_f32_16x16x32_bf16 %[c07], %[fw001], %[fa31], %[c07]\n\t"
+"v_mfma_f32_16x16x32_bf16 %[c14], %[fw011], %[fa01], %[c14]\n\t"
+"v_mfma_f32_16x16x32_bf16 %[c15], %[fw011], %[fa11], %[c15]\n\t"
+"v_mfma_f32_16x16x32_bf16 %[c16], %[fw011], %[fa21], %[c16]\n\t"
+"v_mfma_f32_16x16x32_bf16 %[c17], %[fw011], %[fa31], %[c17]\n\t"
+"s_setprio 0\n\t"
+"s_barrier\n\t"
+"s_sub_i32 %[n], %[n], 1\n\t"
+"s_cmp_lg_u32 %[n], 0\n\t"
+"s_cbranch_scc0 .Lpp16_end_%=\n\t"
+"ds_read_b128 %[fa00], %[la10] offset:0\n\t"
+"ds_read_b128 %[fa01], %[la11] offset:0\n\t"
+"ds_read_b128 %[fa10], %[la10] offset:2048\n\t"
+"ds_read_b128 %[fa11], %[la11] offset:2048\n\t"
+"ds_read_b128 %[fa20], %[la10] offset:4096\n\t"
+"ds_read_b128 %[fa21], %[la11] offset:4096\n\t"
+"ds_read_b128 %[fa30], %[la10] offset:6144\n\t"
+"ds_read_b128 %[fa31], %[la11] offset:6144\n\t"
+"ds_read_b128 %[fw000], %[lw10] offset:0\n\t"
+"ds_read_b128 %[fw001], %[lw11] offset:0\n\t"
+"ds_read_b128 %[fw010], %[lw10] offset:2048\n\t"
+"ds_read_b128 %[fw011], %[lw11] offset:2048\n\t"
+"s_mov_b32 m0, %[ma00]\n\t"
+"s_nop 0\n\t"
+"global_load_lds_dwordx4 %[oa00], s[80:81]\n\t"
+"s_mov_b32 m0, %[ma01]\n\t"
+"s_nop 0\n\t"
+"global_load_lds_dwordx4 %[oa01], s[80:81]\n\t"
+"s_waitcnt vmcnt(4)\n\t"
+"s_waitcnt lgkmcnt(0)\n\t"
+"s_barrier\n\t"
+"s_setprio 1\n\t"
+"v_mfma_f32_16x16x32_bf16 %[c00], %[fw000], %[fa00], %[c00]\n\t"
+"v_mfma_f32_16x16x32_bf16 %[c01], %[fw000], %[fa10], %[c01]\n\t"
+"v_mfma_f32_16x16x32_bf16 %[c02], %[fw000], %[fa20], %[c02]\n\t"
+"v_mfma_f32_16x16x32_bf16 %[c03], %[fw000], %[fa30], %[c03]\n\t"
+"v_mfma_f32_16x16x32_bf16 %[c10], %[fw010], %[fa00], %[c10]\n\t"
+"v_mfma_f32_16x16x32_bf16 %[c11], %[fw010], %[fa10], %[c11]\n\t"
+"v_mfma_f32_16x16x32_bf16 %[c12], %[fw010], %[fa20], %[c12]\n\t"
+"v_mfma_f32_16x16x32_bf16 %[c13], %[fw010], %[fa30], %[c13]\n\t"
+"v_mfma_f32_16x16x32_bf16 %[c00], %[fw001], %[fa01], %[c00]\n\t"
+"v_mfma_f32_16x16x32_bf16 %[c01], %[fw001], %[fa11], %[c01]\n\t"
+"v_mfma_f32_16x16x32_bf16 %[c02], %[fw001], %[fa21], %[c02]\n\t"
+"v_mfma_f32_16x16x32_bf16 %[c03], %[fw001], %[fa31], %[c03]\n\t"
+"v_mfma_f32_16x16x32_bf16 %[c10], %[fw011], %[fa01], %[c10]\n\t"
+"v_mfma_f32_16x16x32_bf16 %[c11], %[fw011], %[fa11], %[c11]\n\t"
+"v_mfma_f32_16x16x32_bf16 %[c12], %[fw011], %[fa21], %[c12]\n\t"
+"v_mfma_f32_16x16x32_bf16 %[c13], %[fw011], %[fa31], %[c13]\n\t"
+"s_setprio 0\n\t"
+"s_barrier\n\t"
+"ds_read_b128 %[fw100], %[lw10] offset:4096\n\t"
+"ds_read_b128 %[fw101], %[lw11] offset:4096\n\t"
+"ds_read_b128 %[fw110], %[lw10] offset:6144\n\t"
+"ds_read_b128 %[fw111], %[lw11] offset:6144\n\t"
+"s_mov_b32 m0, %[mw00]\n\t"
+"s_nop 0\n\t"
+"global_load_lds_dwordx4 %[ow00], s[82:83]\n\t"
+"s_mov_b32 m0, %[mw01]\n\t"
+"s_nop 0\n\t"
+"global_load_lds_dwordx4 %[ow01], s[82:83]\n\t"
+"s_waitcnt vmcnt(4)\n\t"
+"s_waitcnt lgkmcnt(0)\n\t"
+"s_barrier\n\t"
+"s_setprio 1\n\t"
+"v_mfma_f32_16x16x32_bf16 %[c20], %[fw100], %[fa00], %[c20]\n\t"
+"v_mfma_f32_16x16x32_bf16 %[c21], %[fw100], %[fa10], %[c21]\n\t"
+"v_mfma_f32_16x16x32_bf16 %[c22], %[fw100], %[fa20], %[c22]\n\t"
+"v_mfma_f32_16x16x32_bf16 %[c23], %[fw100], %[fa30], %[c23]\n\t"
+"v_mfma_f32_16x16x32_bf16 %[c30], %[fw110], %[fa00], %[c30]\n\t"
+"v_mfma_f32_16x16x32_bf16 %[c31], %[fw110], %[fa10], %[c31]\n\t"
+"v_mfma_f32_16x16x32_bf16 %[c32], %[fw110], %[fa20], %[c32]\n\t"
+"v_mfma_f32_16x16x32_bf16 %[c33], %[fw110], %[fa30], %[c33]\n\t"
+"v_mfma_f32_16x16x32_bf16 %[c20], %[fw101], %[fa01], %[c20]\n\t"
+"v_mfma_f32_16x16x32_bf16 %[c21], %[fw101], %[fa11], %[c21]\n\t"
+"v_mfma_f32_16x16x32_bf16 %[c22], %[fw101], %[fa21], %[c22]\n\t"
+"v_mfma_f32_16x16x32_bf16 %[c23], %[fw101], %[fa31], %[c23]\n\t"
+"v_mfma_f32_16x16x32_bf16 %[c30], %[fw111], %[fa01], %[c30]\n\t"
+"v_mfma_f32_16x16x32_bf16 %[c31], %[fw111], %[fa11], %[c31]\n\t"
+"v_mfma_f32_16x16x32_bf16 %[c32], %[fw111], %[fa21], %[c32]\n\t"
+"v_mfma_f32_16x16x32_bf16 %[c33], %[fw111], %[fa31], %[c33]\n\t"
+"s_setprio 0\n\t"
+"s_barrier\n\t"
+"ds_read_b128 %[fa00], %[la10] offset:8192\n\t"
+"ds_read_b128 %[fa01], %[la11] offset:8192\n\t"
+"ds_read_b128 %[fa10], %[la10] offset:10240\n\t"
+"ds_read_b128 %[fa11], %[la11] offset:10240\n\t"
+"ds_read_b128 %[fa20], %[la10] offset:12288\n\t"
+"ds_read_b128 %[fa21], %[la11] offset:12288\n\t"
+"ds_read_b128 %[fa30], %[la10] offset:14336\n\t"
+"ds_read_b128 %[fa31], %[la11] offset:14336\n\t"
+"s_mov_b32 m0, %[mw10]\n\t"
+"s_nop 0\n\t"
+"global_load_lds_dwordx4 %[ow10], s[82:83]\n\t"
+"s_mov_b32 m0, %[mw11]\n\t"
+"s_nop 0\n\t"
+"global_load_lds_dwordx4 %[ow11], s[82:83]\n\t"
+"s_add_u32 s82, s82, %[wk]\n\t"
+"s_addc_u32 s83, s83, 0\n\t"
+"s_waitcnt vmcnt(4)\n\t"
+"s_waitcnt lgkmcnt(0)\n\t"
+"s_barrier\n\t"
+"s_setprio 1\n\t"
+"v_mfma_f32_16x16x32_bf16 %[c24], %[fw100], %[fa00], %[c24]\n\t"
+"v_mfma_f32_16x16x32_bf16 %[c25], %[fw100], %[fa10], %[c25]\n\t"
+"v_mfma_f32_16x16x32_bf16 %[c26], %[fw100], %[fa20], %[c26]\n\t"
+"v_mfma_f32_16x16x32_bf16 %[c27], %[fw100], %[fa30], %[c27]\n\t"
+"v_mfma_f32_16x16x32_bf16 %[c34], %[fw110], %[fa00], %[c34]\n\t"
+"v_mfma_f32_16x16x32_bf16 %[c35], %[fw110], %[fa10], %[c35]\n\t"
+"v_mfma_f32_16x16x32_bf16 %[c36], %[fw110], %[fa20], %[c36]\n\t"
+"v_mfma_f32_16x16x32_bf16 %[c37], %[fw110], %[fa30], %[c37]\n\t"
+"v_mfma_f32_16x16x32_bf16 %[c24], %[fw101], %[fa01], %[c24]\n\t"
+"v_mfma_f32_16x16x32_bf16 %[c25], %[fw101], %[fa11], %[c25]\n\t"
+"v_mfma_f32_16x16x32_bf16 %[c26], %[fw101], %[fa21], %[c26]\n\t"
+"v_mfma_f32_16x16x32_bf16 %[c27], %[fw101], %[fa31], %[c27]\n\t"
+"v_mfma_f32_16x16x32_bf16 %[c34], %[fw111], %[fa01], %[c34]\n\t"
+"v_mfma_f32_16x16x32_bf16 %[c35], %[fw111], %[fa11], %[c35]\n\t"
+"v_mfma_f32_16x16x32_bf16 %[c36], %[fw111], %[fa21], %[c36]\n\t"
+"v_mfma_f32_16x16x32_bf16 %[c37], %[fw111], %[fa31], %[c37]\n\t"
+"s_setprio 0\n\t"
+"s_barrier\n\t"
+"s_mov_b32 m0, %[ma10]\n\t"
+"s_nop 0\n\t"
+"global_load_lds_dwordx4 %[oa10], s[80:81]\n\t"
+"s_mov_b32 m0, %[ma11]\n\t"
+"s_nop 0\n\t"
+"global_load_lds_dwordx4 %[oa11], s[80:81]\n\t"
+"s_add_u32 s80, s80, %[ak]\n\t"
+"s_addc_u32 s81, s81, 0\n\t"
+"s_waitcnt vmcnt(4)\n\t"
+"s_waitcnt lgkmcnt(0)\n\t"
+"s_barrier\n\t"
+"s_setprio 1\n\t"
+"v_mfma_f32_16x16x32_bf16 %[c04], %[fw000], %[fa00], %[c04]\n\t"
+"v_mfma_f32_16x16x32_bf16 %[c05], %[fw000], %[fa10], %[c05]\n\t"
+"v_mfma_f32_16x16x32_bf16 %[c06], %[fw000], %[fa20], %[c06]\n\t"
+"v_mfma_f32_16x16x32_bf16 %[c07], %[fw000], %[fa30], %[c07]\n\t"
+"v_mfma_f32_16x16x32_bf16 %[c14], %[fw010], %[fa00], %[c14]\n\t"
+"v_mfma_f32_16x16x32_bf16 %[c15], %[fw010], %[fa10], %[c15]\n\t"
+"v_mfma_f32_16x16x32_bf16 %[c16], %[fw010], %[fa20], %[c16]\n\t"
+"v_mfma_f32_16x16x32_bf16 %[c17], %[fw010], %[fa30], %[c17]\n\t"
+"v_mfma_f32_16x16x32_bf16 %[c04], %[fw001], %[fa01], %[c04]\n\t"
+"v_mfma_f32_16x16x32_bf16 %[c05], %[fw001], %[fa11], %[c05]\n\t"
+"v_mfma_f32_16x16x32_bf16 %[c06], %[fw001], %[fa21], %[c06]\n\t"
+"v_mfma_f32_16x16x32_bf16 %[c07], %[fw001], %[fa31], %[c07]\n\t"
+"v_mfma_f32_16x16x32_bf16 %[c14], %[fw011], %[fa01], %[c14]\n\t"
+"v_mfma_f32_16x16x32_bf16 %[c15], %[fw011], %[fa11], %[c15]\n\t"
+"v_mfma_f32_16x16x32_bf16 %[c16], %[fw011], %[fa21], %[c16]\n\t"
+"v_mfma_f32_16x16x32_bf16 %[c17], %[fw011], %[fa31], %[c17]\n\t"
+"s_setprio 0\n\t"
+"s_barrier\n\t"
+"s_sub_i32 %[n], %[n], 1\n\t"
+"s_cmp_lg_u32 %[n], 0\n\t"
+"s_cbranch_scc1 .Lpp16_loop_%=\n\t"
+".Lpp16_end_%=:\n\t"
+"s_waitcnt lgkmcnt(0)\n\t"
+"s_nop 7\n\t"
+"s_nop 7\n\t"
+"s_nop 3\n\t"
```
